# scipopt/SCIP-SDP

Measured on AMD Instinct MI355X. Metric: node-SDP solves/sec, dense block n x n with m vars (IPM iters/sec in iters_per_sec), higher is better.
Workload: dtype f64

## Files before the change

include/hipsdp.h:

```cpp
#ifndef HIPSDP_H
#define HIPSDP_H

#ifdef __cplusplus
extern "C" {
#endif

#define HIPSDP_API __attribute__((visibility("default")))

#define HIPSDP_OK             0
#define HIPSDP_ERR_NODEVICE   1
#define HIPSDP_ERR_HIP        2
#define HIPSDP_ERR_ARG        3
#define HIPSDP_ERR_NOMEM      4
#define HIPSDP_ERR_NUMERIC    5

#define HIPSDP_STATUS_OPTIMAL   0
#define HIPSDP_STATUS_DINF      1
#define HIPSDP_STATUS_DUNB      2
#define HIPSDP_STATUS_PDINF     3
#define HIPSDP_STATUS_ITERLIM   4
#define HIPSDP_STATUS_NUMERIC   5
#define HIPSDP_STATUS_TIMELIM   6
#define HIPSDP_STATUS_OBJLIM    7
#define HIPSDP_STATUS_UNSOLVED -1
// ... 27 lines not shown
   double dinf;
   double dabs;
   double gap;
   double mu;
   double tau, kappa;
   double solve_seconds;
   double schur_seconds;
   double schur_flops;
   int    schur_calls;
   int    chol_fail;
   int    warm_started;
   int    settings_used;
   double schur_flops_executed;
} hipsdp_info;

HIPSDP_API const char* hipsdp_last_error(void);
HIPSDP_API const char* hipsdp_version(void);
HIPSDP_API int  hipsdp_device_count(void);
HIPSDP_API void hipsdp_default_params(hipsdp_params* p);

HIPSDP_API int  hipsdp_create(hipsdp_solver** solver, int device);
HIPSDP_API void hipsdp_free(hipsdp_solver** solver);

HIPSDP_API int  hipsdp_set_shape(hipsdp_solver* solver, int m, int nblocks, const int* blocksizes, int q);
HIPSDP_API int  hipsdp_set_shape2(hipsdp_solver* solver, int m, int nblocks, const int* blocksizes, int q, const long long* nnz);
HIPSDP_API int  hipsdp_block_is_sparse(hipsdp_solver* solver, int block);
HIPSDP_API int  hipsdp_sparse_policy(hipsdp_solver* solver, int mode);
HIPSDP_API int  hipsdp_func_attr_sets(int device);
HIPSDP_API int  hipsdp_mem_info(int device, double* free_bytes, double* total_bytes);
HIPSDP_API int  hipsdp_set_obj(hipsdp_solver* solver, const double* b);
HIPSDP_API int  hipsdp_add_entries(hipsdp_solver* solver, int block, long long nnz, const int* var, const int* row, const int* col,
   const double* val);
HIPSDP_API int  hipsdp_master_define(hipsdp_solver* solver, int nvars, int nblocks, const int* blocksizes, const int* nblockvars);
HIPSDP_API int  hipsdp_master_add_entries(hipsdp_solver* solver, int block, long long nnz, const int* slot, const int* row, const int* col,
   const double* val);
HIPSDP_API int  hipsdp_master_add_vars(hipsdp_solver* solver, int block, int nslots, const int* nnz, const int* const* row,
   const int* const* col, const double* const* val);
HIPSDP_API int  hipsdp_master_gather(hipsdp_solver* solver, int engine_block, int master_block, int nactive, const int* slots,
   int nkept, const int* kept);
HIPSDP_API int  hipsdp_master_define2(hipsdp_solver* solver, int nvars, int nblocks, const int* blocksizes, const int* nblockvars,
   const long long* nnz);
HIPSDP_API int  hipsdp_master_block_is_sparse(hipsdp_solver* solver, int master_block);
HIPSDP_API int  hipsdp_master_gather_stats(hipsdp_solver* solver, long long* device_builds, long long* host_builds, long long* launches,
   long long* readbacks);
HIPSDP_API int  hipsdp_set_block_dense(hipsdp_solver* solver, int block, const double* A);
HIPSDP_API int  hipsdp_set_lp(hipsdp_solver* solver, const double* Dext);
HIPSDP_API int  hipsdp_block_device_ptr(hipsdp_solver* solver, int block, double** dptr);

HIPSDP_API int  hipsdp_set_start(hipsdp_solver* solver, const double* y, const double* const* X, const double* const* Z,
   const double* x, const double* z);

HIPSDP_API int  hipsdp_solve(hipsdp_solver* solver, const hipsdp_params* params, hipsdp_info* info);
HIPSDP_API int  hipsdp_gram_cache_stats(hipsdp_solver* solver, long long* hits, long long* misses);

HIPSDP_API int  hipsdp_solve_path(hipsdp_solver* solver);
HIPSDP_API long long hipsdp_solve1_solves(void);
HIPSDP_API long long hipsdp_solve1_fallbacks(void);
HIPSDP_API long long hipsdp_solve1_fallbacks_warm(void);
HIPSDP_API int hipsdp_solve1_debug_counts(unsigned int* counts2);
HIPSDP_API int  hipsdp_solve1_trace(hipsdp_solver* solver, double* out64, int maxrows, double* hist);

HIPSDP_API int hipsdp_solve_many(int count, hipsdp_solver* const* solvers, const hipsdp_params* params,
                                 hipsdp_info* infos, int* rcs);
HIPSDP_API int hipsdp_solve_many_stats(long long* launches, long long* problems);

HIPSDP_API int hipsdp_solve_objectives(hipsdp_solver* solver, int count, const double* B, const hipsdp_params* params,
                                       hipsdp_info* infos, double* Y, int* rcs);
HIPSDP_API int hipsdp_solve_objectives_stats(long long* calls, long long* launches, long long* problems);

HIPSDP_API int  hipsdp_get_y(hipsdp_solver* solver, double* y);
HIPSDP_API int  hipsdp_get_X(hipsdp_solver* solver, int block, double* X);
HIPSDP_API int  hipsdp_get_Z(hipsdp_solver* solver, int block, double* Z);
HIPSDP_API int  hipsdp_get_lp(hipsdp_solver* solver, double* x, double* z);
HIPSDP_API int  hipsdp_get_preoptimal(hipsdp_solver* solver, int* available, double* y, double* x);
HIPSDP_API int  hipsdp_get_preoptimal_X(hipsdp_solver* solver, int block, double* X);

HIPSDP_API int  hipsdp_check_y(hipsdp_solver* solver, const double* y, double* lmin, double* lpviol);
HIPSDP_API int  hipsdp_check_y_tol(hipsdp_solver* solver, const double* y, double tol, double* lmin, double* lpviol);

HIPSDP_API int  hipsdp_sync_flag(hipsdp_solver* solver, int* flag);

#define HIPSDP_NPHASES 7
HIPSDP_API int  hipsdp_set_profiling(hipsdp_solver* solver, int on);
HIPSDP_API int  hipsdp_get_phase_times(hipsdp_solver* solver, double* ms );
HIPSDP_API const char* hipsdp_phase_name(int phase);

HIPSDP_API int  hipsdp_eigencuts(hipsdp_solver* solver, int block, const double* y, double tol, int maxcuts, int* ncuts, double* eigvals,
                      double* coefs, double* lhs, double* vecs);
HIPSDP_API int hipsdp_eigencuts_all(hipsdp_solver* solver, const double* y, double tol, int maxcuts, int* ncuts, double* lmin,
                                    double* eigvals, double* coefs, double* lhs, double* vecs);
HIPSDP_API int hipsdp_eigencuts_all_stats(long long* calls, long long* launches, long long* readbacks);

#define HIPSDP_SPARSECUTS_MAXIT 10000
typedef struct hipsdp_sparsecut_opts {
   double tol;
   double feastol;
   double convtol;
   int    maxcuts;
   int    maxit;
} hipsdp_sparsecut_opts;
HIPSDP_API int hipsdp_sparsecuts_all(hipsdp_solver* solver, const double* y, const int* sizes, const hipsdp_sparsecut_opts* opts,
   int* ncuts, double* lmin, double* eigvals, double* coefs, double* lhs, double* vecs, int* iters, int* flags);
HIPSDP_API int hipsdp_sparsecuts_all_stats(long long* calls, long long* launches, long long* readbacks);

#define HIPSDP_SPARSECUTS_MAXN 512
HIPSDP_API int hipsdp_sparsecuts(hipsdp_solver* solver, int block, const double* y, int size, const hipsdp_sparsecut_opts* opts,
// ... 102 lines not shown
```

include/hipsdp_units.h:

```cpp
#ifndef HIPSDP_UNITS_H
#define HIPSDP_UNITS_H

#include "hipsdp.h"

#ifdef __cplusplus
extern "C" {
#endif

HIPSDP_API int  hipsdp_dgemm_selfcheck(int device, int M, int N, int K, int layB, int batch, int splitk, int flags, double beta,
   int* used_v2, long long* ndiff);
HIPSDP_API int  hipsdp_pass_at_unit(int device, int R, long long E, const double* A, const double* coef, double sa, const double* add, int split,
   double* out, int* chunks);
HIPSDP_API int  hipsdp_dgemm_selfcheck2(int device, int M, int N, int K, int layB, int batch, int splitk, int flags, double alpha, double beta,
   int reps, int* used, long long* ndiff, double* ms_tile, double* ms_fast);
HIPSDP_API int  hipsdp_gram_plan_info(int device, int M, long long K, int nslab, int* no, int* nd, int* nitems, double* span);
HIPSDP_API int  hipsdp_gram_selfcheck(int device, int M, long long K, int reps, int* used, double* maxdiff, long long* nrepro, double* ms_tile,
   double* ms_gram);
HIPSDP_API int  hipsdp_dgemm_selfcheck3(int device, int M, int N, int K, int layB, int batch, int splitk, int flags, double alpha, double beta,
   int reps, int* used, long long* ndiff, double* maxdiff, long long* nrepro, double* ms_tile, double* ms_fast);
HIPSDP_API int  hipsdp_tri_product_unit(int device, int mode, int M, int N, int K, int layB, int batch, int flags, const double* A,
   const double* B, double* Cio, int crows, int ldc, int* used);
HIPSDP_API int  hipsdp_tri_instance_force(int mode);
HIPSDP_API int  hipsdp_schur_identity_unit(int device, int m1, int n, const double* A, double ws_gbytes, int full_storage, double* Mx,
   double* flops);
// ... 30 lines not shown
   double* dZ);
HIPSDP_API int  hipsdp_tail_dirmat_unit(int device, int n, int fused, double s1, const double* Zinv, const double* X, const double* GZ, double* H,
   double* pk);
HIPSDP_API int  hipsdp_tail_sc_len(void);
HIPSDP_API int  hipsdp_tail_dir_unit(int device, int m, int n, int fused, const double* B, const double* H, const double* rhs2, const double* rp,
   const double* b, const double* u1, const double* u2, const double* par, double* sc, double* dy, double* dyt);
HIPSDP_API int  hipsdp_tail_dots_unit(int device, int m, int n, int fused, const double* a, const double* v, double* out);
HIPSDP_API int  hipsdp_trtri(int device, int n, const double* A, double* Linv);
HIPSDP_API int  hipsdp_lambda_min(int device, int n, const double* W, int steps, double* theta, double* resid);
HIPSDP_API int  hipsdp_lambda_min_scaled(int device, int n, const double* L, const double* D, int steps, double* theta, double* resid);
HIPSDP_API int  hipsdp_solve1_fits(int m, int q, int nblk, const int* ns);
HIPSDP_API int  hipsdp_solve1_class(int m, int nblk, const int* ns);
HIPSDP_API unsigned long long hipsdp_gram_gen_next(unsigned long long* counter);
HIPSDP_API int  hipsdp_gram_key_match_unit(int m_a, int nblk_a, const int* n_a, const int* form_a, const unsigned long long* gen_a,
   const long long* ws_a, int m_b, int nblk_b, const int* n_b, const int* form_b, const unsigned long long* gen_b, const long long* ws_b);
HIPSDP_API int  hipsdp_syev_many_unit(int device, int count, const int* ns, const double* A, double* lam, double* V, int* launches);
HIPSDP_API int  hipsdp_sparsecuts_unit(int device, int count, const int* ns, const double* Z, const double* v0, const double* maxeig,
   const int* sizes, const hipsdp_sparsecut_opts* opts, int* ncuts, double* eigvals, double* vecs, int* iters, int* flags);
HIPSDP_API int  hipsdp_sparsecuts_large_unit(int device, int n, const double* Z, const double* v0, double maxeig, int size,
   const hipsdp_sparsecut_opts* opts, int* ncuts, double* eigvals, double* vecs, int* iters, int* flags);
HIPSDP_API int  hipsdp_tridiag_unit(int device, int n, const double* A, double* d, double* e, double* Vrefl, double* tau);
HIPSDP_API int  hipsdp_tvec_unit(int device, int n, const double* d, const double* e, double* lam, double* Z);
HIPSDP_API int  hipsdp_sparse_dump_unit(hipsdp_solver* solver, int block, long long* counts, int* voff, int* vrow, int* vcol, double* vval,
   int* poff, int* prow, int* pcol, int* pvar, double* pval, int* foff, int* frow, int* fcol, double* fval, int* soff, int* srow, int* sent);
HIPSDP_API int  hipsdp_onevar_unit(int device, int n, int count, const double* Z, const double* A, const double* shift, const int* kind,
   const double* lb, const double* ub, double feastol, int maxevals, int* status, double* optval, double* lmin, double* grad, int* evals);
HIPSDP_API int  hipsdp_onevar_all_unit(int device, int count, const int* n, const double* Z, const double* A, const double* shift,
   const int* kind, const double* lb, const double* ub, double feastol, int maxevals, int mid_cap,
   int* status, double* optval, double* lmin, double* grad, int* evals);
HIPSDP_API int  hipsdp_onevar_large_unit(int device, int count, const int* n, const double* Z, const double* A, const double* shift,
   const int* kind, const double* lb, const double* ub, double feastol, int maxevals, int wg_cap, int chunk,
   int* status, double* optval, double* lmin, double* grad, int* evals, int* rounds);
HIPSDP_API int  hipsdp_objs_fanout_unit(int device, int count, int m, int q, int nblk, const int* ns, const double* B, const double* b_own,
   int have_start, const double* y, const double* x, const double* z, const double* XZ, int gap, double guard, long long* lane_len,
   long long* offs, double* lanes, int* launches);
HIPSDP_API int  hipsdp_small_dir_block_unit(int device, int n, double c, double s1, const double* X, const double* R, const double* E,
   const double* Zinv, int recorded, double* out, int* pending);
HIPSDP_API int  hipsdp_small_lp_rows_unit(int device, int q, int m1, const double* Dext, const double* v, int mode, double eta, double sigmu,
   const double* x, const double* z, const double* rd, const double* elp, int recorded, double* out1, double* out2, int* pending);
HIPSDP_API int  hipsdp_small_apply_A_unit(int device, int m1, int nblk, const int* n2, const double* A, const double* V, int q,
   const double* Dext, const double* vlp, int epi, double scal, const double* vin, int recorded, double* out, double* vout, int* pending);
HIPSDP_API int  hipsdp_small_elementwise_unit(int device, int n, const int* nn, const double* par, int use_elp, const double* in,
   const double* xs, int recorded, double* o_lp, double* o_mul, double* o_ext, double* ys, int* pending);
HIPSDP_API int  hipsdp_small_gemv_t_unit(int device, int R, long long E, long long lda, const double* A, const double* coef, double sa,
   int add_mode, const double* add, int recorded, double* out, int* pending);
HIPSDP_API int  hipsdp_reductions_unit(int device, int kind, int count, const int* len, const int* slot, const int* accumulate,
   const double* a, const double* b, const double* c, int nslots, const double* preset, int recorded, double* out, int* pending);
HIPSDP_API int  hipsdp_small_solve_unit(int device, int m, const double* M, int form, int nrhs, long long ld, double* rhs, double* u2,
   double* wt, int* pending, int* fail);
HIPSDP_API int  hipsdp_gemv_t3_unit(int device, int R, long long E, long long lda, const double* A, const double* c, int fused, double* out,
   int* took);
HIPSDP_API int  hipsdp_pass_a_unit(int device, int R, long long E, long long lda, const double* A, int nv, const double* V, int voff,
   long long wsdoubles, double* out, int* info);

#ifdef __cplusplus
}
#endif

#endif
```

scip-sdp_amd/binding.py:

```python
import ctypes as C
import os
import numpy as np

_HERE = os.path.dirname(os.path.abspath(__file__))
LIBPATH = os.environ.get("HIPSDP_LIB", os.path.join(_HERE, "lib", "libhipsdp.so"))

STATUS_NAMES = {0: "optimal", 1: "dual_infeasible", 2: "dual_unbounded", 3: "both_infeasible", 4: "iterlimit",
                5: "numeric", 6: "timelimit", 7: "objlimit", -1: "unsolved"}


class Params(C.Structure):
    _fields_ = [("gaptol", C.c_double), ("feastol", C.c_double), ("infeastol", C.c_double), ("objlimit", C.c_double),
                ("timelimit", C.c_double), ("gamma", C.c_double), ("ws_gbytes", C.c_double), ("maxiter", C.c_int),
                ("verbose", C.c_int), ("lanczos_steps", C.c_int), ("settings", C.c_int), ("pabstol", C.c_double), ("preoptgap", C.c_double)]


class Info(C.Structure):
    _fields_ = [("status", C.c_int), ("iterations", C.c_int), ("pobj", C.c_double), ("dobj", C.c_double),
                ("pinf", C.c_double), ("dinf", C.c_double), ("dabs", C.c_double), ("gap", C.c_double), ("mu", C.c_double),
                ("tau", C.c_double), ("kappa", C.c_double), ("solve_seconds", C.c_double), ("schur_seconds", C.c_double),
                ("schur_flops", C.c_double), ("schur_calls", C.c_int), ("chol_fail", C.c_int), ("warm_started", C.c_int),
                ("settings_used", C.c_int), ("schur_flops_executed", C.c_double)]


# ... 202 lines not shown
        A = np.zeros((self.m + 1, self.ns[k], self.ns[k]))
        _chk(self._l().hipsdp_get_block_dense(self.h, k, _dp(A)), "hipsdp_get_block_dense")
        return A

    def load_core(self, prob):
        self.set_shape(prob.m, [A.shape[1] for A in prob.blocks], prob.q)
        self.set_obj(prob.b)
        for k, A in enumerate(prob.blocks):
            self.set_block_dense(k, A)
        if prob.q:
            self.set_lp(np.concatenate([np.asarray(prob.c).reshape(-1, 1), prob.D], axis=1))

    def set_start(self, y, X, Z, x=None, z=None):
        y = _f64(y)
        Xs = [_f64(M) for M in X]
        Zs = [_f64(M) for M in Z]
        PX = (C.POINTER(C.c_double) * max(len(Xs), 1))(*[_dp(M) for M in Xs])
        PZ = (C.POINTER(C.c_double) * max(len(Zs), 1))(*[_dp(M) for M in Zs])
        xx = _f64(x if x is not None else np.zeros(max(self.q, 1)))
        zz = _f64(z if z is not None else np.zeros(max(self.q, 1)))
        _chk(self._l().hipsdp_set_start(self.h, _dp(y), PX, PZ, _dp(xx), _dp(zz)), "hipsdp_set_start")

    def solve(self, **kw):
        p = Params()
        self._l().hipsdp_default_params(C.byref(p))
        for k, v in kw.items():
            setattr(p, k, v)
        info = Info()
        _chk(self._l().hipsdp_solve(self.h, C.byref(p), C.byref(info)), "hipsdp_solve")
        return info

    def solve_objectives(self, B, **kw):
        B = _f64(B)
        if B.ndim != 2 or B.shape[1] != self.m:
            raise ValueError("solve_objectives: B must be count x %d" % self.m)
        n = B.shape[0]
        p = _params(kw)
        infos = (Info * max(n, 1))()
        rcs = (C.c_int * max(n, 1))()
        Y = np.zeros((n, self.m))
        rc = self._l().hipsdp_solve_objectives(self.h, n, _dp(B), C.byref(p), infos, _dp(Y), rcs)
        if rc != 0:
            raise RuntimeError("hipsdp_solve_objectives failed: rc=%d, per job %s (%s)" %
                               (rc, list(rcs)[:n], self._l().hipsdp_last_error().decode()))
        return [infos[i] for i in range(n)], Y

    def solve_path(self):
        return self._l().hipsdp_solve_path(self.h)

    def gram_cache_stats(self):
        hits = C.c_longlong(0)
        misses = C.c_longlong(0)
        _chk(self._l().hipsdp_gram_cache_stats(self.h, C.byref(hits), C.byref(misses)), "hipsdp_gram_cache_stats")
        return hits.value, misses.value

    def solve1_trace(self, rows=0):
        out = np.zeros(64)
        hist = np.zeros((max(rows, 1), 16))
        _chk(self._l().hipsdp_solve1_trace(self.h, _dp(out), rows, _dp(hist) if rows else None), "hipsdp_solve1_trace")
        return out, hist[:rows]

    def y(self):
        out = np.zeros(self.m)
        _chk(self._l().hipsdp_get_y(self.h, _dp(out)), "hipsdp_get_y")
        return out

    def X(self, k):
        out = np.zeros((self.ns[k], self.ns[k]))
        _chk(self._l().hipsdp_get_X(self.h, k, _dp(out)), "hipsdp_get_X")
        return out

    def Z(self, k):
        out = np.zeros((self.ns[k], self.ns[k]))
        _chk(self._l().hipsdp_get_Z(self.h, k, _dp(out)), "hipsdp_get_Z")
        return out

    def lp(self):
        x = np.zeros(self.q)
        z = np.zeros(self.q)
        _chk(self._l().hipsdp_get_lp(self.h, _dp(x), _dp(z)), "hipsdp_get_lp")
        return x, z

    def preoptimal(self):
        avail = C.c_int(0)
        y = np.zeros(max(1, self.m))
        x = np.zeros(max(1, self.q))
        _chk(self._l().hipsdp_get_preoptimal(self.h, C.byref(avail), _dp(y), _dp(x)), "hipsdp_get_preoptimal")
        if not avail.value:
            return None
        Xs = []
        for k, n in enumerate(self.ns):
            X = np.zeros((n, n))
            _chk(self._l().hipsdp_get_preoptimal_X(self.h, k, _dp(X)), "hipsdp_get_preoptimal_X")
            Xs.append(X)
        return y[:self.m], Xs, x[:self.q]

    def check_y(self, y, tol=0.0):
        y = _f64(y)
        lmin = np.zeros(max(1, len(self.ns)))
        viol = C.c_double(0.0)
        if tol > 0.0:
            _chk(self._l().hipsdp_check_y_tol(self.h, _dp(y), C.c_double(tol), _dp(lmin), C.byref(viol)), "hipsdp_check_y_tol")
        else:
            _chk(self._l().hipsdp_check_y(self.h, _dp(y), _dp(lmin), C.byref(viol)), "hipsdp_check_y")
        return lmin[:len(self.ns)], viol.value

# ... 516 lines not shown
def schur_sparse_unit2(n, m, coo, X, Zinv, kernel=-1, device=0):
    var, row, col, val = _coo_i32(coo)
    X = _f64(X); Zinv = _f64(Zinv)
    Mx = np.zeros((m + 1, m + 1))
    took = C.c_int(-7)
    _chk(ulib().hipsdp_schur_sparse_unit2(device, n, m, C.c_longlong(len(val)), _ip(var), _ip(row), _ip(col), _dp(val), _dp(X), _dp(Zinv),
                                          _dp(Mx), int(kernel), C.byref(took)), "hipsdp_schur_sparse_unit2")
    return Mx, took.value


def sparse_ops_unit(n, m, coo, V=None, coef=None, base=None, device=0):
    var, row, col, val = _coo_i32(coo)
    outA = outAT = None
    pV = pc = pb = pA = pAT = None
    if V is not None:
        V = _f64(V)
        assert V.shape == (n, n)
        outA = np.full(m, np.nan)
        pV, pA = _dp(V), _dp(outA)
    if coef is not None:
        coef = _f64(coef)
        assert coef.shape == (m + 1,)
        base = np.zeros((n, n)) if base is None else _f64(base)
        assert base.shape == (n, n)
        outAT = np.full((n, n), np.nan)
        pc, pb, pAT = _dp(coef), _dp(base), _dp(outAT)
    _chk(ulib().hipsdp_sparse_ops_unit(device, n, m, C.c_longlong(len(val)), _ip(var), _ip(row), _ip(col), _dp(val), pV, pc, pb, pA, pAT),
         "hipsdp_sparse_ops_unit")
    return outA, outAT


def schur_w(A, X, Z, device=0):
    A = _f64(A)
    m1, n = A.shape[0], A.shape[1]
    X = _f64(X)
    Z = _f64(Z)
    Mx = np.zeros((m1, m1))
    _chk(ulib().hipsdp_schur_w(device, m1, n, _dp(A), _dp(X), _dp(Z), _dp(Mx)), "hipsdp_schur_w")
    return Mx


def schur_form_unit(form, A, P, Q, parts=1, ws_gbytes=0.0, device=0):
    A = _f64(A)
    m1, n = A.shape[0], A.shape[1]
    P = _f64(P); Q = _f64(Q)
    assert A.shape == (m1, n, n) and P.shape == (n, n) and Q.shape == (n, n)
    Mx = np.zeros((m1, m1))
    used = (C.c_int * 3)(0, 0, 0)
    _chk(ulib().hipsdp_schur_form_unit(device, form, parts, m1, n, _dp(A), _dp(P), _dp(Q), C.c_double(ws_gbytes), _dp(Mx), used),
         "hipsdp_schur_form_unit")
    return Mx, tuple(used)


def schur_small_unit(As, Xs, Zinvs, Dext=None, x=None, z=None, fill=0.0, device=0):
    As = [_f64(a) for a in As]; Xs = [_f64(a) for a in Xs]; Zinvs = [_f64(a) for a in Zinvs]
    nblk, m1 = len(As), As[0].shape[0]
    ns = np.array([a.shape[1] for a in As], dtype=np.int32)
    for k in range(nblk):
        assert As[k].shape == (m1, ns[k], ns[k]) and Xs[k].shape == (ns[k], ns[k]) and Zinvs[k].shape == (ns[k], ns[k])
    q = 0 if Dext is None else int(np.shape(Dext)[0])
    if q > 0:
        Dext = _f64(Dext); x = _f64(x); z = _f64(z)
        assert Dext.shape == (q, m1) and x.shape == (q,) and z.shape == (q,)
    arr = C.POINTER(C.c_double) * nblk
    pA, pX, pZ = arr(*[_dp(a) for a in As]), arr(*[_dp(a) for a in Xs]), arr(*[_dp(a) for a in Zinvs])
    m = m1 - 1
    Mx = np.full((m1, m1), fill)
    Lm = np.full(max(m * m, 1), fill)
    dg = np.full(max(m, 1), fill)
    taken = C.c_int(-1)
    _chk(ulib().hipsdp_schur_small_unit(device, m1, nblk, _ip(ns), pA, pX, pZ, q, _dp(Dext) if q else None, _dp(x) if q else None,
                                        _dp(z) if q else None, _dp(Mx), _dp(Lm), _dp(dg), C.byref(taken)), "hipsdp_schur_small_unit")
    return taken.value, Mx, Lm[:m * m].reshape(m, m), dg[:m]


def gram_plan_info(M, K, nslab=64, device=0):
    no, nd, ni = C.c_int(0), C.c_int(0), C.c_int(0)
    sp = C.c_double(0.0)
    rc = ulib().hipsdp_gram_plan_info(device, M, C.c_longlong(K), nslab, C.byref(no), C.byref(nd), C.byref(ni), C.byref(sp))
    return (no.value, nd.value, ni.value, sp.value) if rc == 0 else None


def dgemm_selfcheck(M, N, K, layB=1, batch=1, splitk=1, flags=0, beta=0.0, device=0):
    used = C.c_int(0)
    nd = C.c_longlong(0)
    _chk(ulib().hipsdp_dgemm_selfcheck(device, M, N, K, layB, batch, splitk, flags, C.c_double(beta), C.byref(used), C.byref(nd)),
         "hipsdp_dgemm_selfcheck")
    return used.value, nd.value


def dgemm_selfcheck2(M, N, K, layB=1, batch=1, splitk=1, flags=0, alpha=1.0, beta=0.0, reps=0, device=0):
    used = C.c_int(0)
    nd = C.c_longlong(0)
    t0, t1 = C.c_double(0.0), C.c_double(0.0)
    _chk(ulib().hipsdp_dgemm_selfcheck2(device, M, N, K, layB, batch, splitk, flags, C.c_double(alpha), C.c_double(beta), reps,
                                       C.byref(used), C.byref(nd), C.byref(t0), C.byref(t1)), "hipsdp_dgemm_selfcheck2")
    return used.value, nd.value, t0.value, t1.value


def dgemm_selfcheck3(M, N, K, layB=1, batch=1, splitk=1, flags=0, alpha=1.0, beta=0.0, reps=0, device=0):
    used = C.c_int(0)
    nd, nr = C.c_longlong(0), C.c_longlong(0)
    md, t0, t1 = C.c_double(0.0), C.c_double(0.0), C.c_double(0.0)
    _chk(ulib().hipsdp_dgemm_selfcheck3(device, M, N, K, layB, batch, splitk, flags, C.c_double(alpha), C.c_double(beta), reps,
                                       C.byref(used), C.byref(nd), C.byref(md), C.byref(nr), C.byref(t0), C.byref(t1)), "hipsdp_dgemm_selfcheck3")
    return used.value, nd.value, md.value, nr.value, t0.value, t1.value
# ... 236 lines not shown
    _chk(ulib().hipsdp_small_elementwise_unit(device, n, _ip(nn), _dp(par), int(use_elp), _dp(vecs), _dp(xs), int(recorded), _dp(o_lp),
                                              _dp(o_mul), _dp(o_ext), _dp(ys), C.byref(pend)), "hipsdp_small_elementwise_unit")
    return o_lp, o_mul, o_ext, ys, pend.value


def small_gemv_t_unit(A, E, coef, sa, add, add_mode, recorded, device=0):
    A, coef = _f64(A), _f64(coef)
    R, lda = A.shape
    add = None if add is None else _f64(add)
    assert coef.size == R and 1 <= E <= lda and (add_mode == 0 or add.size == E)
    out, pend = np.zeros(E), C.c_int(-1)
    _chk(ulib().hipsdp_small_gemv_t_unit(device, R, C.c_longlong(E), C.c_longlong(lda), _dp(A), _dp(coef), C.c_double(sa), int(add_mode),
                                         _opt(add), int(recorded), _dp(out), C.byref(pend)), "hipsdp_small_gemv_t_unit")
    return out, pend.value


def reductions_unit(kind, lens, slots, accumulate, a, b, c, preset, recorded, device=0):
    lens, slots, accumulate = (np.ascontiguousarray(v, dtype=np.int32) for v in (lens, slots, accumulate))
    a, b, c, preset = _f64(a), _f64(b), _f64(c), _f64(preset)
    assert lens.size == slots.size == accumulate.size and a.size == b.size == c.size == int(lens.sum())
    out, pend = np.zeros(preset.size), C.c_int(-1)
    _chk(ulib().hipsdp_reductions_unit(device, int(kind), lens.size, _ip(lens), _ip(slots), _ip(accumulate), _dp(a), _dp(b), _dp(c),
                                       preset.size, _dp(preset), int(recorded), _dp(out), C.byref(pend)), "hipsdp_reductions_unit")
    return out, pend.value


def small_solve_unit(M, rhs, form, ld=None, device=0):
    M = _f64(M)
    m = M.shape[0]
    rhs = _f64(rhs).copy()
    pend, fail = C.c_int(-1), C.c_int(-1)
    if form == 0:
        nrhs, ld = rhs.shape
        _chk(ulib().hipsdp_small_solve_unit(device, m, _dp(M), 0, nrhs, C.c_longlong(ld), _dp(rhs), None, None, C.byref(pend),
                                            C.byref(fail)), "hipsdp_small_solve_unit")
        return rhs, pend.value, fail.value
    assert rhs.size == 2 * m
    u2, wt = np.zeros(m), np.zeros(m + 1)
    _chk(ulib().hipsdp_small_solve_unit(device, m, _dp(M), 1, 0, C.c_longlong(0), _dp(rhs), _dp(u2), _dp(wt), C.byref(pend),
                                        C.byref(fail)), "hipsdp_small_solve_unit")
    return rhs, u2, wt, fail.value


def gemv_t3_unit(A, E, c, fused, device=0):
    A, c = _f64(A), _f64(c)
    R, lda = A.shape
    assert c.shape == (3, R) and 1 <= E <= lda
    out, took = np.zeros((3, E)), C.c_int(-1)
    _chk(ulib().hipsdp_gemv_t3_unit(device, R, C.c_longlong(E), C.c_longlong(lda), _dp(A), _dp(c), int(fused), _dp(out), C.byref(took)),
         "hipsdp_gemv_t3_unit")
    return out, took.value


def pass_a_unit(A, E, V, voff=0, wsdoubles=0, device=0):
    A, V = _f64(A), _f64(V)
    R, lda = A.shape
    nv = V.shape[0]
    assert V.shape == (nv, E) and 1 <= E <= lda
    out = np.zeros((nv, R))
    info = np.zeros(2, dtype=np.int32)
    _chk(ulib().hipsdp_pass_a_unit(device, R, C.c_longlong(E), C.c_longlong(lda), _dp(A), nv, _dp(V), int(voff), C.c_longlong(wsdoubles),
                                   _dp(out), _ip(info)), "hipsdp_pass_a_unit")
    return out, int(info[0]), bool(info[1])


def trtri(A, device=0):
    A = _f64(A)
    Li = np.zeros_like(A)
    _chk(ulib().hipsdp_trtri(device, A.shape[0], _dp(A), _dp(Li)), "hipsdp_trtri")
    return Li


def lambda_min(W, steps=0, device=0):
    W = _f64(W)
    th = C.c_double(0.0)
    rs = C.c_double(0.0)
    _chk(ulib().hipsdp_lambda_min(device, W.shape[0], _dp(W), steps, C.byref(th), C.byref(rs)), "hipsdp_lambda_min")
    return th.value, rs.value


def syev(A, device=0):
    A = _f64(A)
    n = A.shape[0]
    lam = np.zeros(n)
    V = np.zeros((n, n))
    _chk(lib().hipsdp_syev(device, n, _dp(A), _dp(lam), _dp(V)), "hipsdp_syev")
    return lam, V


def syevx(A, il, iu, vectors=True, device=0):
    A = _f64(A)
    n = A.shape[0]
    k = max(0, iu - il + 1)
    lam = np.zeros(k)
    V = np.zeros((k, n)) if vectors else None
    _chk(lib().hipsdp_syevx(device, n, _dp(A), int(il), int(iu), _dp(lam), _dp(V) if vectors else None), "hipsdp_syevx")
    return lam, V


def syevx_below(A, bound, maxk, vectors=True, device=0):
    A = _f64(A)
    n = A.shape[0]
    lam = np.zeros(max(1, maxk))
    V = np.zeros((max(1, maxk), n)) if vectors else None
    cnt, nbelow = C.c_int(-1), C.c_int(-1)
    _chk(lib().hipsdp_syevx_below(device, n, _dp(A), C.c_double(bound), int(maxk), C.byref(cnt), C.byref(nbelow), _dp(lam),
# ... 97 lines not shown
```

scip-sdp_amd/csrc/chol.hip:

```cpp
#include "hs_kernels.h"
#include "hs_wave.h"
#include <cstdlib>

#define NB 64

#ifdef PD_TIMING
__device__ long long pd_tbuf[16];
__device__ int pd_tj0;
#define PD_T(idx) do { if ( threadIdx.x == 0 && j0 == pd_tj0 && blockIdx.x == (gridDim.x > 1 ? 1u : 0u) ) pd_tbuf[idx] = wall_clock64(); } while (0)
extern "C" __attribute__((visibility("default"))) int hipsdp_debug_pd_timing(int j0, long long* out)
{
   if ( out != NULL && hipMemcpyFromSymbol(out, HIP_SYMBOL(pd_tbuf), sizeof(long long) * 16) != hipSuccess )
      return 1;
   return hipMemcpyToSymbol(HIP_SYMBOL(pd_tj0), &j0, sizeof(int)) == hipSuccess ? 0 : 1;
}
#else
#define PD_T(idx) do { } while (0)
#endif

__device__ __forceinline__ void sqrt_and_rsqrt(double d, double y0, double* sd, double* isd)
{
   const double t = d * y0;
   const double e = fma(-t, y0, 1.0);
   const double p = fma(0.375, e, 0.5);
   const double y = fma(y0 * e, p, y0);
   double g = d * y;
   g = fma(fma(-g, g, d), 0.5 * y, g);
   *sd = g;
   *isd = y;
}

__device__ __forceinline__ void pd_wave_sync()
{
   __builtin_amdgcn_fence(__ATOMIC_RELEASE, "wavefront");
   __builtin_amdgcn_wave_barrier();
   __builtin_amdgcn_fence(__ATOMIC_ACQUIRE, "wavefront");
}

struct __attribute__((aligned(16))) dpair { double x, y; };
typedef double v4dc __attribute__((ext_vector_type(4)));

#define PD_LD (NB + 2)
#define PD_SMEM_BYTES ((2 * NB * PD_LD + 5 * NB) * (int) sizeof(double))

struct pd_ext
{
   const double* base;
   const double* dir;
   double        alpha;
   double*       Mout;
   double*       Linv;
   double*       Gram;
   int           set_flag;
   int           rule;
   int*          regmask;
   int           from_lds;
   int           nostore;
   double*       Lout;
};

__device__ __forceinline__ void pd_load_panel(double (&r)[16], const double (*W)[PD_LD], int lane, int c0, bool mine)
{
#pragma unroll
   for (int q = 0; q < 8; ++q)
   {
      dpair u = {0.0, 0.0};
      if ( mine )
         u = *reinterpret_cast<const dpair*>(&W[lane][c0 + 2 * q]);
      r[2 * q] = u.x;
      r[2 * q + 1] = u.y;
   }
}

template<bool CHECKED>
__device__ __forceinline__ bool pd_panel(double (&r)[16], const double (&thr)[16], const double* __restrict__ d0s, int lane, int c0, int nb, int j0,
   bool psd, double regtol, int rule, double (&isdo)[16], unsigned& fbits, int& bad, double* __restrict__ colb)
{
   bool special = false;
   fbits = 0u;
   double cprev[16], tprev = 0.0;
   double d = hs_lane(r[0], c0);
#pragma unroll
   for (int k = 0; k < 16; ++k)
   {
      const int gk = c0 + k;
      const double a = r[k];
      double sa = 0.0, sb = 0.0, sa2 = 0.0;
      if ( k + 1 < 16 )
      {
         sa = hs_lane(a, gk + 1);
         sb = hs_lane(r[k + 1], gk + 1);
      }
      if ( k + 2 < 16 )
         sa2 = hs_lane(a, gk + 2);
      double rc0 = __builtin_amdgcn_rcp(d);
      double y0 = __builtin_amdgcn_rsq(d);
// ... 577 lines not shown
         bufB[row][col] = v;
      }
   __syncthreads();
   ps_mma<true>(bufB, bufA, wave, lane, acc);
#pragma unroll
   for (int t = 0; t < 4; ++t)
#pragma unroll
      for (int rr = 0; rr < 4; ++rr)
      {
         const int row = 16 * wave + lk + 4 * rr, col = 16 * t + lr;
         if ( row < rows )
            Ark[(long long) row * lda + col] = forced[col] != 0.0 ? 0.0 : acc[t][rr];
      }
   PD_T(10);
}

template<int NBK>
__global__ void __launch_bounds__(256) k_potrf_step(double* __restrict__ A, long long lda, int n, int kb, int nblk,
   double* __restrict__ dinv, int* __restrict__ flag, const double* __restrict__ diag0, double regtol, pd_ext ext)
{
   ps_step_body<NBK>(A, lda, n, kb, nblk, dinv, flag, diag0, regtol, ext);
}

struct ps_job { double* A; double* dinv; int* flag; };
template<int NBK>
__global__ void __launch_bounds__(256) k_potrf_step_pair(ps_job J0, ps_job J1, long long lda, int n, int kb, int nblk, pd_ext ext)
{
   const ps_job J = blockIdx.y ? J1 : J0;
   ps_step_body<NBK>(J.A, lda, n, kb, nblk, J.dinv, J.flag, NULL, 1e-13, ext);
}

template<int NBK>
static int launch_potrf_step_pair(hipStream_t s, const ps_job* J, long long lda, int n, int kb, int nblk, const pd_ext& ext)
{
   static hs_attr_mask attr_done;
   HS_CALL( hs_func_max_lds(reinterpret_cast<const void*>(&k_potrf_step_pair<NBK>), PD_SMEM_BYTES, &attr_done) );
   const int nS = nblk - kb;
   const int t = nblk - kb - 1;
   const int nT = kb > 0 ? t * (t + 1) / 2 : 0;
   hipLaunchKernelGGL((k_potrf_step_pair<NBK>), dim3(nS + nT, 2), dim3(256), PD_SMEM_BYTES, s, J[0], J[1], lda, n, kb, nblk, ext);
   HS_LAUNCH_CHECK();
   return HS_OK;
}

template<int NBK>
static int launch_potrf_step(hipStream_t s, double* A, long long lda, int n, int kb, int nblk, double* dinv, int* flag,
   const double* diag0, const pd_ext& ext)
{
   static hs_attr_mask attr_done;
   HS_CALL( hs_func_max_lds(reinterpret_cast<const void*>(&k_potrf_step<NBK>), PD_SMEM_BYTES, &attr_done) );
   const int nS = nblk - kb;
   const int t = nblk - kb - 1;
   const int nT = kb > 0 ? t * (t + 1) / 2 : 0;
   hipLaunchKernelGGL((k_potrf_step<NBK>), dim3(nS + nT), dim3(256), PD_SMEM_BYTES, s, A, lda, n, kb, nblk, dinv, flag, diag0, 1e-13, ext);
   HS_LAUNCH_CHECK();
   return HS_OK;
}

template<int NBK>
static int launch_potrf_diag(hipStream_t s, double* Ajj, long long lda, int nb, int j0, double* dj, int* flag, const double* diag0,
   const pd_ext* extp = NULL)
{
   pd_ext ext = {NULL, NULL, 0.0, NULL, NULL, NULL, 0, 2, NULL};
   if ( extp != NULL )
      ext = *extp;
   static hs_attr_mask attr_done;
   HS_CALL( hs_func_max_lds(reinterpret_cast<const void*>(&k_potrf_diag<NBK>), PD_SMEM_BYTES, &attr_done) );
   hipLaunchKernelGGL((k_potrf_diag<NBK>), dim3(1), dim3(256), PD_SMEM_BYTES, s, Ajj, lda, nb, j0, dj, flag, diag0, 1e-13, ext);
   HS_LAUNCH_CHECK();
   return HS_OK;
}

int hs_potrf_small_ext(hipStream_t s, int n, double* L, double* dinv, int* flag, const double* base, const double* dir, double alpha,
   double* Mout, double* Linv, double* Gram, int set_flag)
{
   if ( n <= 0 )
      return HS_OK;
   if ( n > NB || base == NULL || (Gram != NULL && n > 32) )
      return HS_ERR_ARG;
   pd_ext ext = {base, dir, alpha, Mout, Linv, Gram, set_flag, 2, NULL};
   if ( n <= 16 )
      return launch_potrf_diag<16>(s, L, n, n, 0, dinv, flag, NULL, &ext);
   if ( n <= 32 )
      return launch_potrf_diag<32>(s, L, n, n, 0, dinv, flag, NULL, &ext);
   if ( n <= 48 )
      return launch_potrf_diag<48>(s, L, n, n, 0, dinv, flag, NULL, &ext);
   return launch_potrf_diag<64>(s, L, n, n, 0, dinv, flag, NULL, &ext);
}

template<int NBK>
static int launch_potrf_diag_pair(hipStream_t s, int n, const pd_job& J0, const pd_job& J1)
{
   static hs_attr_mask attr_done;
   HS_CALL( hs_func_max_lds(reinterpret_cast<const void*>(&k_potrf_diag_pair<NBK>), PD_SMEM_BYTES, &attr_done) );
   hipLaunchKernelGGL((k_potrf_diag_pair<NBK>), dim3(2), dim3(256), PD_SMEM_BYTES, s, J0, J1, (long long) n, n);
   HS_LAUNCH_CHECK();
   return HS_OK;
}

int hs_potrf_small_ext_pair(hipStream_t s, int n, double* const* L, double* const* dinv, int* const* flag, const double* const* base,
   const double* const* dir, double alpha, double* const* Mout, double* const* Linv, double* const* Gram, int set_flag)
{
   if ( n <= 0 )
      return HS_OK;
   if ( n > NB || base[0] == NULL || base[1] == NULL || ((Gram[0] != NULL || Gram[1] != NULL) && n > 32) )
      return HS_ERR_ARG;
   pd_job J[2];
   for (int k = 0; k < 2; ++k)
   {
      const pd_ext ext = {base[k], dir[k], alpha, Mout[k], Linv[k], Gram[k], set_flag, 2, NULL};
      J[k].A = L[k]; J[k].dinv = dinv[k]; J[k].flag = flag[k]; J[k].ext = ext;
   }
   if ( n <= 16 )
      return launch_potrf_diag_pair<16>(s, n, J[0], J[1]);
   if ( n <= 32 )
      return launch_potrf_diag_pair<32>(s, n, J[0], J[1]);
   if ( n <= 48 )
      return launch_potrf_diag_pair<48>(s, n, J[0], J[1]);
   return launch_potrf_diag_pair<64>(s, n, J[0], J[1]);
}

__global__ void k_zero_forced_cols(int rows, int nb, double* __restrict__ P, long long lda, const int* __restrict__ mask)
{
   for (long long e = (long long) blockIdx.x * blockDim.x + threadIdx.x; e < (long long) rows * nb; e += (long long) gridDim.x * blockDim.x)
   {
      const int r = (int) (e / nb), c = (int) (e - (long long) r * nb);
      if ( mask[c] )
         P[(long long) r * lda + c] = 0.0;
   }
}

static int g_potrf_force_v1 = 0;
int hs_potrf_force_v1(int on) { const int old = g_potrf_force_v1; g_potrf_force_v1 = on; return old; }

long long hs_potrf_dinv_len(int n)
{
   const long long nblk = n > 0 ? (n + NB - 1) / NB : 1;
   return (nblk > 1 ? 2 : 1) * nblk * NB * NB;
}

int hs_potrf(hipStream_t s, int n, double* A, double* dinv, int* flag, const double* diag0)
{
   return hs_potrf_psd(s, n, A, dinv, flag, diag0, NULL, 0);
}

int hs_potrf_pair(hipStream_t s, int n, const hs_potrf_job* jobs)
{
   if ( n <= 0 )
      return HS_OK;
   if ( jobs == NULL || jobs[0].A == NULL || jobs[1].A == NULL || jobs[0].A == jobs[1].A || jobs[0].dinv == jobs[1].dinv )
      return HS_ERR_ARG;
   const int nblk = (n + NB - 1) / NB;
   if ( nblk <= 1 || g_potrf_force_v1 )
   {
      HS_CALL( hs_potrf(s, n, jobs[0].A, jobs[0].dinv, jobs[0].flag, NULL) );
      return hs_potrf(s, n, jobs[1].A, jobs[1].dinv, jobs[1].flag, NULL);
   }
   const ps_job J[2] = {{jobs[0].A, jobs[0].dinv, jobs[0].flag}, {jobs[1].A, jobs[1].dinv, jobs[1].flag}};
   const pd_ext est = {NULL, NULL, 0.0, NULL, NULL, NULL, 0, 3, NULL, 0, 0, NULL};
   for (int b = 0; b < nblk; ++b)
   {
      const int nb = (n - b * NB) < NB ? (n - b * NB) : NB;
      if ( nb <= 16 )
         HS_CALL( launch_potrf_step_pair<16>(s, J, n, n, b, nblk, est) );
      else if ( nb <= 32 )
         HS_CALL( launch_potrf_step_pair<32>(s, J, n, n, b, nblk, est) );
      else
         HS_CALL( launch_potrf_step_pair<64>(s, J, n, n, b, nblk, est) );
   }
   return HS_OK;
}

int hs_potrf_psd(hipStream_t s, int n, double* A, double* dinv, int* flag, const double* diag0, int* regmask, int set_flag)
{
   if ( n <= 0 )
      return HS_OK;
   if ( diag0 != NULL && regmask == NULL && n > NB )
      return HS_ERR_ARG;
   static int rule = getenv("HIPSDP_PIVOT_RULE") != NULL ? atoi(getenv("HIPSDP_PIVOT_RULE")) : 3;
   pd_ext ext = {NULL, NULL, 0.0, NULL, NULL, NULL, (set_flag && n <= NB) ? 1 : 0, rule, regmask};
   const pd_ext* extp = ((diag0 != NULL && regmask != NULL) || ext.set_flag) ? &ext : NULL;
   const long long lda = n;
   const int nblk = (n + NB - 1) / NB;
   if ( nblk > 1 && !g_potrf_force_v1 )
   {
      pd_ext est = {NULL, NULL, 0.0, NULL, NULL, NULL, 0, rule, (diag0 != NULL) ? regmask : NULL, 0, 0, NULL};
      for (int b = 0; b < nblk; ++b)
      {
         const int nb = (n - b * NB) < NB ? (n - b * NB) : NB;
         if ( nb <= 16 )
            HS_CALL( launch_potrf_step<16>(s, A, lda, n, b, nblk, dinv, flag, diag0, est) );
         else if ( nb <= 32 )
            HS_CALL( launch_potrf_step<32>(s, A, lda, n, b, nblk, dinv, flag, diag0, est) );
         else
            HS_CALL( launch_potrf_step<64>(s, A, lda, n, b, nblk, dinv, flag, diag0, est) );
      }
      return HS_OK;
   }
   for (int b = 0; b < nblk; ++b)
   {
      const int j0 = b * NB;
      const int nb = (n - j0) < NB ? (n - j0) : NB;
      double* Ajj = A + (long long) j0 * lda + j0;
      double* dj = dinv + (long long) b * NB * NB;
      if ( nb <= 16 )
         HS_CALL( launch_potrf_diag<16>(s, Ajj, lda, nb, j0, dj, flag, diag0, extp) );
      else if ( nb <= 32 )
         HS_CALL( launch_potrf_diag<32>(s, Ajj, lda, nb, j0, dj, flag, diag0, extp) );
      else
         HS_CALL( launch_potrf_diag<64>(s, Ajj, lda, nb, j0, dj, flag, diag0, extp) );
      const int j1 = j0 + nb;
      const int rem = n - j1;
      if ( rem <= 0 )
         break;
      double* P = A + (long long) j1 * lda + j0;
      hs_gemm_args g1 = {rem, nb, nb, HS_KC, HS_KC, P, lda, 0, dj, NB, 0, P, lda, 0, 1.0, 0.0, 1, HS_GEMM_TILE64, 1, NULL};
      HS_CALL( hs_dgemm(s, &g1) );
      if ( diag0 != NULL && regmask != NULL )
      {
         long long blocks = ((long long) rem * nb + 255) / 256;
         if ( blocks > 1024 ) blocks = 1024;
         hipLaunchKernelGGL(k_zero_forced_cols, dim3((unsigned) blocks), dim3(256), 0, s, rem, nb, P, lda, regmask + j0);
         HS_LAUNCH_CHECK();
      }
      double* A22 = A + (long long) j1 * lda + j1;
      hs_gemm_args g2 = {rem, rem, nb, HS_KC, HS_KC, P, lda, 0, P, lda, 0, A22, lda, 0, -1.0, 1.0, 1, HS_GEMM_LOWER | HS_GEMM_TILE64, 1, NULL};
      HS_CALL( hs_dgemm(s, &g2) );
   }
   return HS_OK;
}

__global__ void k_copy_block(const double* __restrict__ src, long long lds_, double* __restrict__ dst, long long ldd, int rows, int cols,
// ... 740 lines not shown
```

scip-sdp_amd/csrc/dgemm2.hip:

```cpp
#include "hs_common.h"
#include <stdlib.h>
#include <map>
#include <mutex>
#include <utility>

typedef double v4d2 __attribute__((ext_vector_type(4)));
typedef __attribute__((address_space(3))) void* hs_lds_ptr;
typedef const __attribute__((address_space(1))) void* hs_gbl_ptr;

#define G2_BT   128
#define G2_BKS  8
#ifndef G2_NS
#define G2_NS   4
#endif
#ifndef G2_WGPC
#define G2_WGPC 2
#endif
#define G2_OPSZ (G2_BT * G2_BKS)
#define G2_SLOT (2 * G2_OPSZ)
#define G2_GPS  4
#ifndef G2_ABL
#define G2_ABL  0
#endif

// ... 1165 lines not shown
      run_band();
      store_item();
      cm0 = nm0; cn0 = nn0; cbz = nbz; cvalid = nvalid;
      ++gi;
   }
   g2_wait_vm<0>();
#ifdef G5_PROF
   if ( lane == 0 )
   {
      unsigned long long* o = g5_prof + ((long long) blockIdx.x * (WIDE ? 8 : 4) + wave) * 8;
      for (int i = 0; i < 7; ++i)
         o[i] = prof_acc[i];
      o[7] = __builtin_readcyclecounter() - prof_t0;
   }
#endif
}

#ifdef G5_PROF
extern "C" __attribute__((visibility("default"))) int hs_dgemm5_prof_read(unsigned long long* out)
{
   return hipMemcpyFromSymbol(out, HIP_SYMBOL(g5_prof), sizeof(unsigned long long) * 512 * 4 * 8) == hipSuccess ? 0 : 1;
}
#endif

static int g2_disabled = 0;
static int g2_taken = 0;
static int g5_taken = 0;
static int g5_wide_mode = -1;
static int g5_wide_taken = 0;

int hs_dgemm2_enable(int on)
{
   g2_disabled = on ? 0 : 1;
   return __atomic_load_n(&g2_taken, __ATOMIC_RELAXED);
}

int hs_dgemm2_paired_taken(void)
{
   return __atomic_load_n(&g5_taken, __ATOMIC_RELAXED);
}

int hs_dgemm2_wide_force(int mode)
{
   if ( mode >= -1 && mode <= 1 )
      g5_wide_mode = mode;
   return __atomic_load_n(&g5_wide_taken, __ATOMIC_RELAXED);
}

int hs_dgemm2_tri5_forced(void)
{
   return g5_wide_mode >= 0;
}

static unsigned int* g5_counters(hipStream_t stream)
{
   static std::mutex mu;
   static std::map<std::pair<int, hipStream_t>, unsigned int*> tab;
   int dev = 0;
   if ( hipGetDevice(&dev) != hipSuccess )
      return NULL;
   std::lock_guard<std::mutex> lk(mu);
   auto it = tab.find(std::make_pair(dev, stream));
   if ( it != tab.end() )
      return it->second;
   unsigned int* q = NULL;
   if ( hipMalloc((void**) &q, 64) != hipSuccess )
      return NULL;
   tab[std::make_pair(dev, stream)] = q;
   return q;
}

int hs_dgemm2_tri5_eligible(const hs_gemm_args* a)
{
   const bool triA = (a->flags & HS_GEMM_A_LOWTRI) != 0, triB = (a->flags & HS_GEMM_B_LOWTRI) != 0;
   return triA != triB && a->splitk <= 1 && !(a->flags & (HS_GEMM_LOWER | HS_GEMM_UPPER | HS_GEMM_A_UPTRI))
      && !(triB && a->layB != HS_MC);
}

int hs_dgemm2_tri5_wide(const hs_gemm_args* a)
{
   if ( !hs_dgemm2_tri5_eligible(a) )
      return 0;
   if ( g5_wide_mode >= 0 )
      return g5_wide_mode;
   const bool triB = (a->flags & HS_GEMM_B_LOWTRI) != 0;
   if ( !((G5_WIDE_TRI >> (triB ? 0 : 1)) & 1) )
      return 0;
   const long long panels = triB ? (a->N + G2_BT - 1) / G2_BT : (a->M + G2_BT - 1) / G2_BT;
   const long long wtiles = triB ? (a->M + 2 * G2_BT - 1) / (2 * G2_BT) : (long long) ((a->N + 2 * G2_BT - 1) / (2 * G2_BT)) * a->batch;
   if ( !triB && 2 * ((a->N + 2 * G2_BT - 1) / (2 * G2_BT)) != (a->N + G2_BT - 1) / G2_BT )
      return 0;
   return panels >= 4 && panels * wtiles >= 256LL * G5_WIDE_MIN_ITEMS;
}

int hs_dgemm2_try(hipStream_t stream, const hs_gemm_args* a, int kchunk)
{
   if ( g2_disabled )
      return 0;
   if ( a->layA != HS_KC || (a->flags & (HS_GEMM_UPPER)) )
      return 0;
   if ( (a->lda & 1) || (a->ldb & 1) || (a->strideA & 1) || (a->strideB & 1) || (a->K & 1) || a->K < 16 )
      return 0;
   if ( (((uintptr_t) a->A) & 15) || (((uintptr_t) a->B) & 15) )
      return 0;
   if ( a->layB == HS_MC && ((a->N & 1) || a->N < 2) )
      return 0;
   if ( (a->flags & HS_GEMM_LOWER) && a->M != a->N )
      return 0;
   if ( a->splitk > 1 && (kchunk & 15) )
      return 0;
   const long long tm = (a->M + G2_BT - 1) / G2_BT, tn = (a->N + G2_BT - 1) / G2_BT;
   const long long ntile = (a->flags & HS_GEMM_LOWER) ? tm * (tm + 1) / 2 : tm * tn;
   const long long nz = a->splitk > 1 ? a->splitk : a->batch;
   const long long total = ntile * nz;
   if ( total < 384 && !(g5_wide_mode >= 0 && hs_dgemm2_tri5_eligible(a)) )
      return 0;
   int grid = 256 * G2_WGPC;
   const int Wx = grid / 8;
   int rotdiv = 0;
   if ( !(a->flags & HS_GEMM_LOWER) )
   {
      if ( (a->flags & HS_GEMM_B_LOWTRI) && tn > 1 && (Wx % tn) == 0 )
         rotdiv = (int) (Wx / tn);
      else if ( (a->flags & (HS_GEMM_A_LOWTRI | HS_GEMM_A_UPTRI)) && tm > 1 && (Wx % (tm * tn)) == 0 )
         rotdiv = (int) (Wx / (tm * tn));
   }
   const size_t smem = (size_t) G2_NS * G2_SLOT * sizeof(double);
   const bool triA = (a->flags & HS_GEMM_A_LOWTRI) != 0, triB = (a->flags & HS_GEMM_B_LOWTRI) != 0;
   if ( hs_dgemm2_tri5_eligible(a) )
   {
      static hs_attr_mask attr5[6];
      const int wide = hs_dgemm2_tri5_wide(a);
      const int inst5 = (triB ? 0 : (a->layB == HS_MC ? 1 : 2)) + 3 * wide;
      const size_t smem5 = (size_t) G5_NS * (wide ? 3 * G2_OPSZ : G2_SLOT) * sizeof(double);
      const void* fn5 = NULL;
      switch ( inst5 )
      {
      case 0: fn5 = reinterpret_cast<const void*>(&hs_dgemm5_kernel<HS_MC, 1, 0>); break;
      case 1: fn5 = reinterpret_cast<const void*>(&hs_dgemm5_kernel<HS_MC, 2, 0>); break;
      case 2: fn5 = reinterpret_cast<const void*>(&hs_dgemm5_kernel<HS_KC, 2, 0>); break;
      case 3: fn5 = reinterpret_cast<const void*>(&hs_dgemm5_kernel<HS_MC, 1, 1>); break;
      case 4: fn5 = reinterpret_cast<const void*>(&hs_dgemm5_kernel<HS_MC, 2, 1>); break;
      default: fn5 = reinterpret_cast<const void*>(&hs_dgemm5_kernel<HS_KC, 2, 1>); break;
      }
      if ( hs_func_max_lds(fn5, (int) smem5, &attr5[inst5]) != HS_OK )
         return -HS_ERR_HIP;
      unsigned int* ctr = g5_counters(stream);
      if ( ctr == NULL || hipMemsetAsync(ctr, 0, 64, stream) != hipSuccess )
         return -HS_ERR_HIP;
      hs_gemm_args a5 = *a;
      a5.flags |= G5_F_NT | G5_F_SETS | G5_F_PAIRS;
      const long long tm5 = triB && wide ? (a->M + 2 * G2_BT - 1) / (2 * G2_BT) : tm;
      const long long tn5 = !triB && wide ? (a->N + 2 * G2_BT - 1) / (2 * G2_BT) : tn;
      const long long ntile5 = tm5 * tn5, total5 = ntile5 * nz;
      const int grid5 = wide ? 256 : grid;
      switch ( inst5 )
      {
      case 0: hipLaunchKernelGGL((hs_dgemm5_kernel<HS_MC, 1, 0>), dim3(grid5), dim3(256), smem5, stream, a5, ntile5, total5, ctr); break;
      case 1: hipLaunchKernelGGL((hs_dgemm5_kernel<HS_MC, 2, 0>), dim3(grid5), dim3(256), smem5, stream, a5, ntile5, total5, ctr); break;
      case 2: hipLaunchKernelGGL((hs_dgemm5_kernel<HS_KC, 2, 0>), dim3(grid5), dim3(256), smem5, stream, a5, ntile5, total5, ctr); break;
      case 3: hipLaunchKernelGGL((hs_dgemm5_kernel<HS_MC, 1, 1>), dim3(grid5), dim3(512), smem5, stream, a5, ntile5, total5, ctr); break;
      case 4: hipLaunchKernelGGL((hs_dgemm5_kernel<HS_MC, 2, 1>), dim3(grid5), dim3(512), smem5, stream, a5, ntile5, total5, ctr); break;
      default: hipLaunchKernelGGL((hs_dgemm5_kernel<HS_KC, 2, 1>), dim3(grid5), dim3(512), smem5, stream, a5, ntile5, total5, ctr); break;
      }
      if ( hipGetLastError() != hipSuccess )
         return -HS_ERR_HIP;
      (void) __atomic_add_fetch(&g2_taken, 1, __ATOMIC_RELAXED);
      (void) __atomic_add_fetch(&g5_taken, 1, __ATOMIC_RELAXED);
      if ( wide )
         (void) __atomic_add_fetch(&g5_wide_taken, 1, __ATOMIC_RELAXED);
      return 1;
   }
   const int il = triA != triB ? (triB ? 1 : 2) : 0;
   static hs_attr_mask attr_done[6];
   const int inst = (a->layB == HS_KC ? 0 : 3) + il;
   const void* fn = NULL;
   switch ( inst )
   {
   case 0: fn = reinterpret_cast<const void*>(&hs_dgemm2_kernel<HS_KC, 0>); break;
   case 1: fn = reinterpret_cast<const void*>(&hs_dgemm2_kernel<HS_KC, 1>); break;
   case 2: fn = reinterpret_cast<const void*>(&hs_dgemm2_kernel<HS_KC, 2>); break;
   case 3: fn = reinterpret_cast<const void*>(&hs_dgemm2_kernel<HS_MC, 0>); break;
   case 4: fn = reinterpret_cast<const void*>(&hs_dgemm2_kernel<HS_MC, 1>); break;
   default: fn = reinterpret_cast<const void*>(&hs_dgemm2_kernel<HS_MC, 2>); break;
   }
   if ( hs_func_max_lds(fn, (int) smem, &attr_done[inst]) != HS_OK )
      return -HS_ERR_HIP;
   switch ( inst )
   {
   case 0: hipLaunchKernelGGL((hs_dgemm2_kernel<HS_KC, 0>), dim3(grid), dim3(256), smem, stream, *a, kchunk, ntile, total, rotdiv); break;
   case 1: hipLaunchKernelGGL((hs_dgemm2_kernel<HS_KC, 1>), dim3(grid), dim3(256), smem, stream, *a, kchunk, ntile, total, rotdiv); break;
   case 2: hipLaunchKernelGGL((hs_dgemm2_kernel<HS_KC, 2>), dim3(grid), dim3(256), smem, stream, *a, kchunk, ntile, total, rotdiv); break;
   case 3: hipLaunchKernelGGL((hs_dgemm2_kernel<HS_MC, 0>), dim3(grid), dim3(256), smem, stream, *a, kchunk, ntile, total, rotdiv); break;
   case 4: hipLaunchKernelGGL((hs_dgemm2_kernel<HS_MC, 1>), dim3(grid), dim3(256), smem, stream, *a, kchunk, ntile, total, rotdiv); break;
   default: hipLaunchKernelGGL((hs_dgemm2_kernel<HS_MC, 2>), dim3(grid), dim3(256), smem, stream, *a, kchunk, ntile, total, rotdiv); break;
   }
   if ( hipGetLastError() != hipSuccess )
      return -HS_ERR_HIP;
   (void) __atomic_add_fetch(&g2_taken, 1, __ATOMIC_RELAXED);
   return 1;
}
```

scip-sdp_amd/csrc/gram.hip:

```cpp
#include "hs_common.h"
#include <stdlib.h>
#include <stdio.h>
#include <map>
#include <mutex>
#include <utility>
#include <tuple>
#include <vector>
#include <queue>
#include <algorithm>
#include <functional>

typedef double gr_v4d __attribute__((ext_vector_type(4)));
typedef __attribute__((address_space(3))) void* gr_lds_ptr;
typedef const __attribute__((address_space(1))) void* gr_gbl_ptr;

#define GR_BT   128
#define GR_BKS  8
#define GR_NS   4
#define GR_OPSZ (GR_BT * GR_BKS)
#define GR_SLOT (2 * GR_OPSZ)
#define GR_GPS  4
#define GR_UNI(x) __builtin_amdgcn_readfirstlane(x)

__device__ __attribute__((aligned(16))) double hs_gr_zero[2] = {0.0, 0.0};
// ... 263 lines not shown
            for (int i = 0; i < 4; ++i)
#pragma unroll
               for (int r = 0; r < 4; ++r)
               {
                  const int row = m0 + wm * 64 + 16 * i + (lane >> 4) + 4 * r;
                  if ( row < g.M )
                  {
                     double* cr = C + (long long) row * g.M + n0 + wn * 64 + (lane & 15);
#pragma unroll
                     for (int j = 0; j < 4; ++j)
                        cr[16 * j] = acc[4 * i + j][r];
                  }
               }
         }
         else
         {
#pragma unroll
            for (int k = 0; k < 9; ++k)
            {
               const int rs = dlo[k] ? wave : 7 - wave;
#pragma unroll
               for (int r = 0; r < 4; ++r)
               {
                  const int row = m0 + 16 * rs + (lane >> 4) + 4 * r;
                  const int col = m0 + 16 * dcol[k] + (lane & 15);
                  if ( row < g.M && col < g.M )
                     C[(long long) row * g.M + col] = acc[k][r];
               }
            }
         }
#pragma unroll
         for (int i = 0; i < 16; ++i)
            acc[i] = (gr_v4d){0.0, 0.0, 0.0, 0.0};
      }
      __syncthreads();
   }
}

__global__ void hs_gram_reduce_kernel(int M, int no, int nd, const double* __restrict__ ws, double* __restrict__ C, long long ldc, double alpha, double beta)
{
   const long long MM = (long long) M * M;
   for (long long e = (long long) blockIdx.x * blockDim.x + threadIdx.x; e < MM; e += (long long) gridDim.x * blockDim.x)
   {
      const int r = (int) (e / M), c = (int) (e - (long long) r * M);
      if ( c > r )
         continue;
      const int ns = (r / GR_BT == c / GR_BT) ? nd : no;
      double s = 0.0;
      for (int k = 0; k < ns; ++k)
         s += ws[(long long) k * MM + e];
      double* q = C + (long long) r * ldc + c;
      *q = beta != 0.0 ? alpha * s + beta * (*q) : alpha * s;
   }
}

namespace {

struct GramPlan
{
   std::vector<gram_item> items;
   std::vector<int> off;
   int no, nd;
   double span;
   double executed;
   gram_item* dev;
   int* devoff;
};

#define GR_DIAG_COST 0.72

bool gr_make_plan(GramPlan& P, int tm, long long K, int so, int sd)
{
   const int noff = tm * (tm - 1) / 2;
   const double cd = GR_DIAG_COST;
   if ( so < 1 || sd < 1 )
      return false;
   long long lo = (K + so - 1) / so, ld = (K + sd - 1) / sd;
   lo = ((lo + GR_BKS - 1) / GR_BKS) * GR_BKS;
   ld = ((ld + GR_BKS - 1) / GR_BKS) * GR_BKS;
   if ( (long long) (so - 1) * lo + 8 * GR_BKS > K || (long long) (sd - 1) * ld + 8 * GR_BKS > K )
      return false;
   std::vector<gram_item> all;
   for (int s = 0; s < so; ++s)
      for (int i = 1; i < tm; ++i)
         for (int j = 0; j < i; ++j)
         {
            gram_item it = {i, j, (int) (s * lo), (int) ((s + 1) * lo < K ? (s + 1) * lo : K), s, 0};
            all.push_back(it);
         }
   for (int s = 0; s < sd; ++s)
      for (int i = 0; i < tm; ++i)
      {
         gram_item it = {i, i, (int) (s * ld), (int) ((s + 1) * ld < K ? (s + 1) * ld : K), s, 0};
         all.push_back(it);
      }
   (void) noff;
   std::stable_sort(all.begin(), all.end(), [](const gram_item& a, const gram_item& b) { return a.k0 < b.k0; });
   auto cost = [&](const gram_item& it) { return (it.ti == it.tj ? cd : 1.0) * (double) (it.k1 - it.k0) / (double) K; };
   double total = 0.0;
   P.executed = 0.0;
   for (const gram_item& it : all)
   {
      total += cost(it);
      P.executed += 2048.0 * (double) ((it.k1 - it.k0 + GR_BKS - 1) / GR_BKS) * (it.ti == it.tj ? 72.0 : 128.0);
   }
   P.items.clear();
// ... 60 lines not shown
         return;
      cand.span += penalty;
      if ( best == NULL || cand.span < best->span )
      {
         if ( best == NULL )
            best = new GramPlan();
         *best = cand;
      }
   };
   const int noff = ntile - tm;
   for (int so = 1; so <= nslab && (long long) noff * so + tm <= 512; ++so)
      for (int sd = (so + 1) / 2; sd <= so && (long long) noff * so + (long long) tm * sd <= 512; ++sd)
         consider(gr_make_plan(cand, tm, K, so, sd), 0.24 * ((double) so * noff + (double) sd * tm) / (double) K);
   if ( best != NULL )
   {
      const int sold = hs_dgemm_pick_xcd_slices(ntile, K);
      const double oldspan = (double) (((long long) ntile * sold + 511) / 512) / (double) sold;
      if ( best->span * 1.03 > oldspan || best->items.size() < 256 )
      {
         delete best;
         best = NULL;
      }
   }
   if ( best != NULL )
   {
      gram_item* d = NULL;
      int* doff = NULL;
      if ( hipMalloc((void**) &d, best->items.size() * sizeof(gram_item)) != hipSuccess
         || hipMemcpy(d, best->items.data(), best->items.size() * sizeof(gram_item), hipMemcpyHostToDevice) != hipSuccess
         || hipMalloc((void**) &doff, 513 * sizeof(int)) != hipSuccess
         || hipMemcpy(doff, best->off.data(), 513 * sizeof(int), hipMemcpyHostToDevice) != hipSuccess )
      {
         if ( d != NULL ) (void) hipFree(d);
         if ( doff != NULL ) (void) hipFree(doff);
         delete best;
         return NULL;
      }
      best->dev = d;
      best->devoff = doff;
   }
   tab[key] = best;
   return best;
}

}

static int gr_taken = 0;

int hs_gram_taken(void)
{
   return __atomic_load_n(&gr_taken, __ATOMIC_RELAXED);
}

int hs_gram_try(hipStream_t stream, int M, long long K, const double* W, long long ldw, double* C, long long ldc, double alpha, double beta,
   double* ws, int nslab, double* executed)
{
   if ( ws == NULL || nslab < 2 || M < 256 || K < 16384 )
      return 0;
   if ( (ldw & 1) || (K & 1) || (((uintptr_t) W) & 15) || K > 2000000000LL )
      return 0;
   if ( nslab > 64 ) nslab = 64;
   GramPlan* P = gr_plan(M, K, nslab);
   if ( P == NULL || P->dev == NULL || P->items.size() < 256 )
      return 0;
   gram_args g;
   g.W = W; g.ldw = ldw; g.M = M; g.ws = ws; g.items = P->dev; g.off = P->devoff;
   static hs_attr_mask attr_done;
   const size_t smem = (size_t) GR_NS * GR_SLOT * sizeof(double);
   if ( hs_func_max_lds(reinterpret_cast<const void*>(&hs_gram_kernel), (int) smem, &attr_done) != HS_OK )
      return -HS_ERR_HIP;
   hipLaunchKernelGGL(hs_gram_kernel, dim3(512), dim3(256), smem, stream, g);
   if ( hipGetLastError() != hipSuccess )
      return -HS_ERR_HIP;
   {
      int blocks = (int) (((long long) M * M + 255) / 256);
      if ( blocks > 2048 ) blocks = 2048;
      hipLaunchKernelGGL(hs_gram_reduce_kernel, dim3(blocks), dim3(256), 0, stream, M, P->no, P->nd, ws, C, ldc, alpha, beta);
      if ( hipGetLastError() != hipSuccess )
         return -HS_ERR_HIP;
   }
   if ( executed != NULL )
      *executed = P->executed;
   (void) __atomic_add_fetch(&gr_taken, 1, __ATOMIC_RELAXED);
   return 1;
}

int hs_gram_plan_info(int M, long long K, int nslab, int* no, int* nd, int* nitems, double* span)
{
   GramPlan* P = gr_plan(M, K, nslab > 64 ? 64 : nslab);
   if ( P == NULL )
      return 0;
   *no = P->no; *nd = P->nd; *nitems = (int) P->items.size(); *span = P->span;
   return 1;
}
```

scip-sdp_amd/csrc/hs_common.h:

```cpp
#ifndef HS_COMMON_H
#define HS_COMMON_H

#include <hip/hip_runtime.h>
#include <stddef.h>
#include <stdint.h>

#define HS_OK            0
#define HS_ERR_NODEVICE  1
#define HS_ERR_HIP       2
#define HS_ERR_ARG       3
#define HS_ERR_NOMEM     4
#define HS_ERR_NUMERIC   5

#define HS_HIP(call)                                                                       \
   do {                                                                                    \
      hipError_t hs_e_ = (call);                                                           \
      if ( hs_e_ != hipSuccess ) {                                                         \
         hs_record_hip_error(hs_e_, #call, __FILE__, __LINE__);                            \
         return (hs_e_ == hipErrorOutOfMemory) ? HS_ERR_NOMEM : HS_ERR_HIP;                \
      }                                                                                    \
   } while (0)

#define HS_CALL(call)                                                                      \
   do {                                                                                    \
// ... 10 lines not shown
         return HS_ERR_HIP;                                                                \
      }                                                                                    \
   } while (0)

void hs_record_hip_error(hipError_t e, const char* what, const char* file, int line);
const char* hs_last_error(void);

struct hs_attr_mask { unsigned long long bits[2]; };
int hs_func_max_lds(const void* fn, int bytes, hs_attr_mask* done);
int hs_func_attr_sets(int device);
int hs_device_cus(void);

int hs_pool_alloc(void** p, size_t bytes);
void hs_pool_free(void* p);
void hs_pool_trim(void);

#define HS_KC 0
#define HS_MC 1

#define HS_GEMM_LOWER     1
#define HS_GEMM_A_LOWTRI  2
#define HS_GEMM_B_LOWTRI  4
#define HS_GEMM_A_UPTRI 256
#define HS_GEMM_XCD       8
#define HS_GEMM_TILE64  128
#define HS_GEMM_NOFAST   64
#define HS_GEMM_UPPER    32
#define HS_GEMM_REMAP    16
int hs_dgemm_pick_xcd_slices(long long ntile, long long K);

struct hs_gemm_args
{
   int            M, N, K;
   int            layA, layB;
   const double*  A;
   long long      lda;
   long long      strideA;
   const double*  B;
   long long      ldb;
   long long      strideB;
   double*        C;
   long long      ldc;
   long long      strideC;
   double         alpha, beta;
   int            batch;
   int            flags;
   int            splitk;
   double*        ws;
};

int hs_dgemm(hipStream_t stream, const hs_gemm_args* args);
int hs_dgemm2_try(hipStream_t stream, const hs_gemm_args* args, int kchunk);
int hs_dgemm2_enable(int on);
int hs_dgemm2_paired_taken(void);
int hs_dgemm2_wide_force(int mode);
int hs_dgemm2_tri5_forced(void);
int hs_gram_taken(void);

int hs_gram_try(hipStream_t stream, int M, long long K, const double* W, long long ldw, double* C, long long ldc, double alpha, double beta,
   double* ws, int nslab, double* executed);
int hs_gram_plan_info(int M, long long K, int nslab, int* no, int* nd, int* nitems, double* span);

int hs_dgemm3_try(hipStream_t stream, const hs_gemm_args* args);

double hs_mfma_flops_total(void);
void   hs_mfma_flops_add(double flops);
int hs_dgemm2_tri5_eligible(const hs_gemm_args* a);
int hs_dgemm2_tri5_wide(const hs_gemm_args* a);
double hs_gemm_executed_flops(const hs_gemm_args* a, int BT, int kstage, int kchunk, int persistent);

int hs_dgemm_pick_splitk(int M, int N, int K, int lowerOnly);

#endif
```

scip-sdp_amd/csrc/hs_gram_cache.h:

```cpp
#ifndef HS_GRAM_CACHE_H
#define HS_GRAM_CACHE_H

#define HS_GRAM_FORM_FULL   1
#define HS_GRAM_FORM_PACKED 2
#define HS_GRAM_MAXBLK 64

struct hs_gram_key
{
   int valid;
   int m, nblk;
   int n[HS_GRAM_MAXBLK];
   int form[HS_GRAM_MAXBLK];
   unsigned long long gen[HS_GRAM_MAXBLK];
   long long kws_len, chunk_cols;
   int ws_full;
};

static inline unsigned long long hs_gen_next(unsigned long long* counter)
{
   return ++*counter;
}

static inline void hs_gram_key_clear(hs_gram_key* k)
{
   k->valid = 0;
   k->m = 0;
   k->nblk = 0;
   k->kws_len = k->chunk_cols = 0;
   k->ws_full = 0;
}

static inline int hs_gram_key_make(hs_gram_key* k, int m, int nblk, const int* n, const int* form, const unsigned long long* gen,
   long long kws_len, long long chunk_cols, int ws_full)
{
   hs_gram_key_clear(k);
   if ( m < 0 || nblk < 1 || nblk > HS_GRAM_MAXBLK )
      return 0;
   for (int b = 0; b < nblk; ++b)
   {
      if ( n[b] < 1 || gen[b] == 0 || (form[b] != HS_GRAM_FORM_FULL && form[b] != HS_GRAM_FORM_PACKED) )
         return 0;
      k->n[b] = n[b];
      k->form[b] = form[b];
      k->gen[b] = gen[b];
   }
   k->m = m;
   k->nblk = nblk;
   k->kws_len = kws_len;
   k->chunk_cols = chunk_cols;
   k->ws_full = ws_full;
   k->valid = 1;
   return 1;
}

static inline int hs_gram_key_match(const hs_gram_key* have, const hs_gram_key* want)
{
   if ( !have->valid || !want->valid || have->m != want->m || have->nblk != want->nblk || have->kws_len != want->kws_len
      || have->chunk_cols != want->chunk_cols || have->ws_full != want->ws_full )
      return 0;
   for (int b = 0; b < have->nblk; ++b)
      if ( have->n[b] != want->n[b] || have->form[b] != want->form[b] || have->gen[b] != want->gen[b] )
         return 0;
   return 1;
}

#endif
```

scip-sdp_amd/csrc/hs_kernels.h:

```cpp
#ifndef HS_KERNELS_H
#define HS_KERNELS_H

#include "hs_common.h"
#include "hs_cut_plan.h"
#include <vector>

int hs_fill(hipStream_t s, double* p, long long n, double v);
int hs_set_identity(hipStream_t s, double* A, int n, double v);
int hs_copy(hipStream_t s, double* dst, const double* src, long long n);
int hs_axpy(hipStream_t s, long long n, double a, const double* x, double* y);
int hs_scale_add(hipStream_t s, long long n, double a, const double* x, double b, const double* y, double* out);
struct hs_trial_job { double* V; const double* dV; double* Vs; double* L; };
int hs_trial_pair(hipStream_t s, long long n, double alpha, int first, const hs_trial_job* jobs);
int hs_mirror_lower(hipStream_t s, double* A, int n, long long lda);
int hs_symmetrize(hipStream_t s, double* A, int n);
int hs_transpose(hipStream_t s, int n, const double* src, double* dst);

int hs_gemv_n(hipStream_t s, int R, long long E, const double* A, long long lda, int nv, const double* const* V,
   double* out, long long ldo, double* ws, long long wsdoubles);
int hs_gemv_t(hipStream_t s, int R, long long E, const double* A, long long lda, const double* coef, double sa,
   const double* add, double* out);

int hs_gemv_t_chunks(int R, long long E);
int hs_gemv_t_ws(hipStream_t s, int R, long long E, const double* A, long long lda, const double* coef, double sa,
// ... 29 lines not shown
#define HS_DOT_SLOT_DOUBLES 256
#define HS_DOT_SLOTS 4
#define HS_RED_WS_DOUBLES (HS_DOT_SLOTS * HS_DOT_SLOT_DOUBLES)
int hs_dot_deferred(hipStream_t s, long long n, const double* a, const double* b, double* out, int accumulate, double* ws, int slot);
int hs_absmax(hipStream_t s, long long n, const double* a, double* out, int accumulate, double* ws);
int hs_ratio_min(hipStream_t s, long long n, const double* x, const double* d, double* out, int accumulate, double* ws);

#define HS_SMALL_N 48
int hs_dir_block_small(hipStream_t s, int n, double c, const double* X, const double* R, const double* E, const double* Zinv,
   double s1, double* out);
int hs_dirmat(hipStream_t s, int n, double s1, const double* Zinv, const double* X, const double* GZ, double* H);
int hs_dirmat_pack(hipStream_t s, int n, double s1, const double* Zinv, const double* X, const double* GZ, double* H, double* pk);

int hs_lp_dir(hipStream_t s, int q, double sigmu, double eta, const double* x, const double* z, const double* rd_or_dz,
   const double* elp, double* out);
int hs_lp_scale_rows(hipStream_t s, int q, int cols, const double* x, const double* z, const double* D, double* S);
int hs_vec_mul(hipStream_t s, long long n, const double* a, const double* b, double* out);
int hs_lp_s0(hipStream_t s, int q, const double* x, const double* z, const double* beta, double* out, int accumulate, double* ws);

int hs_pack_rows(hipStream_t s, int m1, int n, long long Lp, const double* A, double* Apk);
int hs_packed_diag(hipStream_t s, int m1, int n, int ldd, long long Lp, const double* Apk, double* D);
int hs_sub_lower(hipStream_t s, int n, const double* S, double* C);
int hs_pack_weighted(hipStream_t s, int n, const double* V, double* pk);
int hs_unpack_sym(hipStream_t s, int n, const double* pk, double sa, const double* add, double* out);
int hs_unpack_sym3(hipStream_t s, int n, int cnt, const double* const* pk, double* const* out);
int hs_unpack_dz_combine(hipStream_t s, int n, const double* pk, const double* P2, const double* sc, int idtau, double eta, const double* Rd,
   double* dZ);
int hs_zero_upper(hipStream_t s, double* A, int n);

struct hs_schur_ws
{
   double*   T;
   double*   U;
   double*   K;
   double*   V;
   long long capT, capV;
   long long chunk_cols;
   long long n2;
   long long kws_len;
   int       full;
   double*   U2;
   double*   V2;
   void*     evP[2];
   void*     evX[2];
   void*     ev_g2;
   int       (*after_g1)(void*);
   void*     after_g1_arg;
};
int  hs_schur_ws_alloc(hs_schur_ws* w, int m1, long long n2max, double budget_gb);
void hs_schur_ws_free(hs_schur_ws* w);
int  hs_schur_U(hipStream_t s, int m1, int n, const double* A, const double* X, const double* Zinv, double* Mx,
   hs_schur_ws* w, int j_begin, int j_end);
int  hs_schur_W(hipStream_t s, int m1, int n, const double* A, const double* R, const double* G, double* Mx, hs_schur_ws* w);
int  hs_schur_W_identity(hipStream_t s, int m1, int n, const double* A, double* Mx, hs_schur_ws* w);
int  hs_schur_W_identity_range(hipStream_t s, int m1, int n, const double* A, long long k0, long long k1, double* Mx, hs_schur_ws* w);
int  hs_schur_W_identity_packed(hipStream_t s, int m1, int n, const double* Apk, long long Lp, double* Mx, hs_schur_ws* w);
int  hs_schur_identity_packed_fits(const hs_schur_ws* w, int m1, int n);

int  hs_schur_Urows(hipStream_t s, int m1, int n, const double* A, const double* X, const double* Zinv, double* Mx,
   hs_schur_ws* w, int r_begin, int r_end);
void hs_shard_rows(int m1, int nranks, int rank, int* chunk_rows, int* first_begin, int* second_begin);
int  hs_schur_Wcols(hipStream_t s, int m1, int n, const double* A, const double* R, const double* G, double* Mx, hs_schur_ws* w,
   int c0, int cw);
void hs_shard_cols(int m1, int n, int nranks, int rank, int* c_begin, int* c_width);
int  hs_schur_Wvar(hipStream_t s, void* comm, int rank, int nranks, int m1, int n, const double* A, const double* R, const double* G,
   double* Mx, hs_schur_ws* w, int c0, int cw);
int  hs_schur_ws_alloc_var(hs_schur_ws* w, int m1, int nranks, int n, int cwmax);
int  hs_schur_ws_alloc_var_overlap(hs_schur_ws* w);
int  hs_schur_Wvar_all(hipStream_t s, hipStream_t sc, void* comm, int rank, int nranks, int m1, int n, const double* A, const double* R,
   const double* G, double* Mx, hs_schur_ws* w, int cwmax, int overlap);
void hs_var_rows(int m1, int nranks, int rank, int* r0, int* r1);
void hs_var_wrows(int n, int nranks, int rank, int* q0, int* q1);
int  hs_alltoall(void* comm, const double* send, double* recv, const long long* cnt, hipStream_t stream);
int  hs_allreduce_sum(void* comm, double* buf, long long count, hipStream_t stream);
int  hs_mirror_upper(hipStream_t s, double* A, int n, long long lda);
int  hs_allgather_inplace(void* comm, double* buf, long long count_per_rank, int rank, hipStream_t stream);
int  hs_allgather(void* comm, const double* send, double* recv, long long count_per_rank, hipStream_t stream);

struct hs_sparse
{
   int        n, m;
   long long  nnz;
   int*       voff;
   int*       vrow;
   int*       vcol;
   double*    vval;
   long long  npos;
   int*       poff;
   int*       prow;
   int*       pcol;
   int*       pvar;
   double*    pval;
   long long  nfull, nslots;
   int*       foff;
   int*       frow;
   int*       fcol;
   double*    fval;
   int*       soff;
   int*       srow;
   int*       sent;
   double*    Tc;
   int        borrowed;
};
int  hs_sp_prefers_sparse(int n, int m, long long nnz);
int  hs_sp_build(hs_sparse** out, int n, int m, long long nnz, const int* var, const int* row, const int* col, const double* val);
void hs_sp_free(hs_sparse* sp);
long long hs_sp_nnz(const hs_sparse* sp);
int  hs_sp_apply_A(hipStream_t s, const hs_sparse* sp, const double* V, double* out_var1);
int  hs_sp_apply_AT(hipStream_t s, const hs_sparse* sp, const double* coef, double* out);
int  hs_sp_schur(hipStream_t s, const hs_sparse* sp, const double* X, const double* Zinv, double* Mx);
int  hs_sp_schur_ex(hipStream_t s, const hs_sparse* sp, const double* X, const double* Zinv, double* Mx, int kernel, int* took);
int  hs_sp_expand(hipStream_t s, const hs_sparse* sp, double* A);

struct hs_spm;
int  hs_spm_create(hs_spm** out, int N, int S);
void hs_spm_free(hs_spm* M);
int  hs_spm_size(const hs_spm* M);
int  hs_spm_slots(const hs_spm* M);
int  hs_spm_add(hs_spm* M, long long nnz, const int* slot, int oneslot, const int* row, const int* col, const double* val);
int  hs_spm_gather_sparse(hipStream_t s, hs_spm* M, int n, int m, int nactive, const int* act, const int* kept, hs_sparse** out,
   long long* launches, long long* readbacks);
int  hs_spm_gather_dense(hipStream_t s, hs_spm* M, int n, int nactive, const int* dact, const int* dinv, double* A, long long* launches);
struct hipsdp_solver;
int  hs_solver_sparse_block(struct hipsdp_solver* s, int block, const hs_sparse** sp);

struct hs_dir_tail_args { int m, q, K; const int* n; const double* const* B; const double* const* H; const double* beta; const double* hl;
   const double* rhs2; const double* rp; const double* b; double* u1; const double* u2; double* dy; double* dyt; double* sc; double* red_ws;
   const double* dinvm; const double* Lm; double eta, rg, sigmu, tau, kappa, etk; };
int hs_ipm_dir_tail(hipStream_t st, const hs_dir_tail_args* a, int tail, int fuse_solve);
int hs_ipm_after_solve2(hipStream_t st, int m, const double* rhs2, double* u2, double* wt, const double* u1, double* e2, double* e1, int fused);
int hs_ipm_dz_combine(hipStream_t st, long long n2, double* dZ, const double* P2, const double* sc, double eta, const double* Rd);
int hs_ipm_sc_dtau(void);
int hs_ipm_sc_len(int nblocks);

int hs_potrf(hipStream_t s, int n, double* A, double* dinv, int* flag, const double* diag0);
long long hs_potrf_dinv_len(int n);
int hs_potrf_psd(hipStream_t s, int n, double* A, double* dinv, int* flag, const double* diag0, int* regmask, int set_flag);
struct hs_potrf_job { double* A; double* dinv; int* flag; };
int hs_potrf_pair(hipStream_t s, int n, const hs_potrf_job* jobs);
int hs_trtri(hipStream_t s, int n, const double* L, const double* dinv, double* Linv, double* tmp);
int hs_potrf_small_ext_pair(hipStream_t s, int n, double* const* L, double* const* dinv, int* const* flag, const double* const* base,
   const double* const* dir, double alpha, double* const* Mout, double* const* Linv, double* const* Gram, int set_flag);
int hs_potrf_small_ext(hipStream_t s, int n, double* L, double* dinv, int* flag, const double* base, const double* dir, double alpha,
   double* Mout, double* Linv, double* Gram, int set_flag);
int hs_schur_small(hipStream_t s, int m1, int nblk, const int* n, const double* const* A, const double* const* X,
   const double* const* Zinv, int q, const double* Dext, const double* x, const double* z, double* Mx, double* Lm, double* diagM);
int hs_trsv(hipStream_t s, int n, const double* L, const double* dinv, int nrhs, double* rhs, long long ldr, int mode);
long long hs_trsv_sync_ws(int n);
int hs_trsv_sync_init(hipStream_t s, int n, int* sync_ws, int* epoch);
int hs_trsv_sync(hipStream_t s, int n, const double* L, const double* dinv, int nrhs, double* rhs, long long ldr, int mode,
   int* sync_ws, int* epoch);

int hs_lanczos_lmin(hipStream_t s, int n, const double* W, int maxsteps, double* res, double* ws);
long long hs_lanczos_ws(int n, int maxsteps);
#define HS_STEP_MAXJOBS 32
struct hs_step_jobs { int nblk; int n[HS_STEP_MAXJOBS]; const double* L0[HS_STEP_MAXJOBS]; const double* D0[HS_STEP_MAXJOBS];
   const double* L1[HS_STEP_MAXJOBS]; const double* D1[HS_STEP_MAXJOBS]; double* res0[HS_STEP_MAXJOBS]; double* res1[HS_STEP_MAXJOBS]; };
int hs_steplen_small_multi(hipStream_t s, const hs_step_jobs* P, int maxsteps);
int hs_lmin_exact_multi(hipStream_t st, const hs_step_jobs* P);
int hs_lanczos_scaled_small(hipStream_t s, int n, int maxsteps, const double* L0, const double* D0, const double* L1, const double* D1,
   double* res0, double* res1);
int hs_lmin_scaled_tiny(hipStream_t s, int n, const double* L0, const double* D0, const double* L1, const double* D1, double* res0,
   double* res1);
int hs_lanczos_lmin2(hipStream_t s, int n, const double* W0, const double* W1, int maxsteps, double* res0, double* res1,
   double* ws0, double* ws1, int* rot, unsigned long long* dsync, int nwipe);
long long hs_lanczos_sync_words(void);
int hs_lanczos_sync_reset(hipStream_t s, unsigned long long* dsync, int* rot);

long long hs_syev_small_scratch(int n);
int hs_syev_small_dev(hipStream_t st, int n, const double* A, double* lam, double* V, double* scratch);
struct hs_eig_job { int n; int pad; const double* in; double* ws; };
long long hs_syev_many_vecpos(int n);
int hs_syev_many_class(int n);
int hs_syev_small_many(hipStream_t st, int count, const hs_eig_job* hjobs, const hs_eig_job* jobs, int* launches);

int hs_psd_project_one(int device, int n, int nnz, const int* row, const int* col, const double* val, double minev,
   double epsilon, int mode, int cap, int* nnz_out, int* rowout, int* colout, double* valout);

#define HS_EC_DENSE  0
#define HS_EC_PACKED 1
#define HS_EC_SPARSE 2
struct hs_sp_view { long long nnz, npos; const int *voff, *vrow, *vcol; const double* vval; const int *poff, *prow, *pcol, *pvar; const double* pval; };
void hs_sp_get_view(const hs_sparse* sp, hs_sp_view* v);
struct hs_ec_job
{
   int n, form, blk, pad;
   long long ld;
   const double* A;
   hs_sp_view sp;
   double* Z;
// ... 463 lines not shown
```

scip-sdp_amd/csrc/ipm.hip:

```cpp
#include "hs_kernels.h"
#include "hs_gram_cache.h"
#include "hs_sp_master.h"
#include "../../include/hipsdp.h"
#include <rocprofiler-sdk-roctx/roctx.h>
#include <vector>
#include <atomic>
#include <utility>
#include <functional>
#include <chrono>
#include <algorithm>
#include <cmath>
#include <cassert>
#include <cstdio>
#include <cstdlib>
#include <cstring>

enum
{
   SC_AX0 = 0,
   SC_DOBJ,
   SC_XZ,
   SC_RP2,
   SC_RD2,
   SC_RDLPMAX,
// ... 168 lines not shown
   long long gemv_ws_len;
   int* flags;
   hs_schur_ws sws;
   bool schur_mode_U, schur_mode_rows;
   bool schur_mode_cols;
   int  schur_sim_shards;
   bool schur_mode_forced;
   double* Mgather;
   long long mx_rows;
   int nsc;
   bool shaped, solved, have_start;
   int last_status;
   double sol_scale;
   hipEvent_t ev0, ev1;
   int master_nvars;
   std::vector<int> master_sizes;
   std::vector<int> master_slots;
   std::vector<double*> master_A;
   std::vector<hs_spm*> master_sp;
   long long mg_device_builds, mg_host_builds, mg_launches, mg_readbacks;
   void* comm; int rank, nranks;
   double* passg;
   int shard_passes;
   int shardA_req;
   int var_cw;
   bool var_overlap;
   bool shardA;
   int a_r0, a_r1;
   hipsdp_params par;
   PhaseClock pc;
   bool clk_on; unsigned long long* clk_buf; int clk_n; double clk_ghz; hipStream_t clk_stream;
   double* s1_ws;
   long long s1_ws_len;
   double* s1_host;
   double* s1_host_dev;
   bool s1_sol_host;
   bool zero_b, zero_D;
   char* arena_h; char* arena_d; size_t arena_cap, stage_off; bool stage_pending;
   int m_alloc, q_alloc;
   int ncmd;
   hipEvent_t cmd_ev;
   bool cmd_inflight;
   unsigned long long s1_seq;
   int s1_last;
   double* ln_dev; long long ln_dev_len;
   double* ln_host; double* ln_host_dev; long long ln_host_len;
   unsigned long long ln_seq;
   void* stage_h[2]; void* stage_d[2]; hipEvent_t stage_ev[2]; long long stage_cap;
   CutWs cw;
   unsigned long long a_gen_next;
   double* gc_M; long long gc_len; bool gc_nomem;
   hs_gram_key gc_key;
   long long gc_hits, gc_misses;
};

static void a_written(hipsdp_solver* s, Block& B)
{
   B.apk_valid = false;
   B.A_gen = hs_gen_next(&s->a_gen_next);
}

void hs_comm_phase(int phase);

static void phase_mark(hipsdp_solver* s, int ph)
{
   if ( s->pc.open >= 0 )
      (void) roctxRangePop();
   s->pc.open = ph;
   if ( ph >= 0 )
      (void) roctxRangePushA(g_phase_names[ph]);
   if ( !s->pc.on )
      return;
   hipEvent_t e = NULL;
   if ( !s->pc.pool.empty() )
   {
      e = s->pc.pool.back();
      s->pc.pool.pop_back();
   }
   else if ( hipEventCreate(&e) != hipSuccess )
      return;
   if ( hipEventRecord(e, s->stream) == hipSuccess )
      s->pc.marks.push_back(std::make_pair(ph, e));
   else
      s->pc.pool.push_back(e);
}

static void phase_finish(hipsdp_solver* s)
{
   for (size_t i = 0; i + 1 < s->pc.marks.size(); ++i)
   {
      float ms = 0.f;
      const int ph = s->pc.marks[i].first;
      if ( ph >= 0 && hipEventElapsedTime(&ms, s->pc.marks[i].second, s->pc.marks[i + 1].second) == hipSuccess )
         s->pc.ms[ph] += (double) ms;
   }
   for (auto& mk : s->pc.marks)
      s->pc.pool.push_back(mk.second);
   s->pc.marks.clear();
}

extern "C" const char* hipsdp_phase_name(int phase)
{
   return phase >= 0 && phase < PH_COUNT ? g_phase_names[phase] : "";
}

extern "C" int hipsdp_set_profiling(hipsdp_solver* s, int on)
{
// ... 168 lines not shown
      s->zero_b = false;
   }
   if ( s->zero_D )
   {
      HS_CALL( stage_zero(s, s->Dext, (long long) s->q * (s->m + 1)) );
      s->zero_D = false;
   }
   return HIPSDP_OK;
}
static int stage_sync(hipsdp_solver* s)
{
   if ( s != NULL && (s->zero_b || s->zero_D) )
      HS_CALL( flush_zeros(s) );
   if ( s != NULL && s->ncmd > 0 )
      HS_CALL( flush_cmds(s) );
   if ( s != NULL && s->stage_pending )
   {
      HS_HIP( hipStreamSynchronize(s->stream) );
      s->stage_pending = false;
      s->stage_off = 0;
      s->cmd_inflight = false;
   }
   return HIPSDP_OK;
}

static void free_sparse(Block& B)
{
   if ( B.sp != NULL ) hs_sp_free(B.sp);
   B.sp = NULL;
   delete B.sph;
   B.sph = NULL;
}

static void free_problem(hipsdp_solver* s)
{
   if ( s->stream != NULL ) (void) hipStreamSynchronize(s->stream);
   if ( s->stream2 != NULL ) (void) hipStreamSynchronize(s->stream2);
   for (auto& B : s->blk)
   {
      double* ptrs[] = {B.Aown, B.A0sep, B.X, B.Z, B.Rd, B.Lz, B.LzInv, B.Zinv, B.Lx, B.LxInv, B.B, B.H, B.G, B.GZ, B.dXa, B.dZa, B.dX, B.dZ,
         B.E, B.W, B.T1, B.dinvz, B.dinvx, B.Xs, B.Zs, B.Apkown, B.pkv, B.T2, B.W2, B.Xpre, B.P2, B.pk3};
      for (double* p : ptrs) dfree(p);
      free_sparse(B);
   }
   s->blk.clear();
   double* ptrs[] = {s->b, s->Dext, s->y, s->x, s->z, s->yt, s->dyt, s->wt, s->AX, s->AH, s->tmpe, s->rp, s->rd, s->tmpq, s->hl,
      s->beta, s->elp, s->dxa, s->dza, s->dx, s->dz, s->xs, s->zs, s->ys, s->rhs2, s->cvec, s->u2, s->dy, s->dya, s->Mx, s->Lm,
      s->dinvm, s->Slp, s->sc, s->red_ws, s->gemv_ws, s->lan_ws, s->lan_ws2};
   for (double* p : ptrs) dfree(p);
   hs_schur_ws_free(&s->sws);
   if ( s->gc_M != NULL ) (void) hipFree(s->gc_M);
   s->gc_M = NULL; s->gc_len = 0; s->gc_nomem = false;
   hs_gram_key_clear(&s->gc_key);
   if ( s->ln_dev != NULL ) (void) hipFree(s->ln_dev);
   if ( s->ln_host != NULL ) (void) hipHostFree(s->ln_host);
   s->ln_dev = NULL; s->ln_host = NULL; s->ln_host_dev = NULL; s->ln_dev_len = 0; s->ln_host_len = 0;
   dfree(s->Mgather);
   s->Mgather = NULL;
   dfree(s->passg);
   s->passg = NULL;
   dfree(s->trsv_ws);
   s->trsv_ws = NULL;
   dfree(s->gemvt_ws);
   s->gemvt_ws = NULL;
   s->gemvt_ws_len = 0;
   if ( s->lan_sync != NULL )
      (void) hipFree(s->lan_sync);
   s->lan_sync = NULL;
   dfree(s->regmask);
   s->regmask = NULL;
   dfree(s->pre_y); dfree(s->pre_x);
   s->pre_y = s->pre_x = NULL;
   s->pre_valid = false;
   s->b = s->Dext = s->y = s->x = s->z = s->yt = s->dyt = s->wt = s->AX = s->AH = s->tmpe = s->rp = s->rd = s->tmpq = s->hl = NULL;
   s->beta = s->elp = s->dxa = s->dza = s->dx = s->dz = s->xs = s->zs = s->ys = s->u1 = s->rhs2 = s->cvec = s->u2 = s->dy = s->dya = NULL;
   s->Mx = s->Lm = s->dinvm = s->Slp = s->sc = s->red_ws = s->gemv_ws = s->lan_ws = s->lan_ws2 = NULL;
   s->flags = NULL;
   s->shaped = false;
   s->solved = false;
}

extern "C" int hipsdp_create(hipsdp_solver** out, int device)
{
   g_err[0] = 0;
   int nd = hipsdp_device_count();
   if ( nd <= 0 )
   {
      set_err("no HIP device available (hipsdp has no CPU fallback)");
      return HIPSDP_ERR_NODEVICE;
   }
   if ( device < 0 || device >= nd )
      return HIPSDP_ERR_ARG;
   HS_HIP( hipSetDevice(device) );
   hipsdp_solver* s = new hipsdp_solver();
   memset((void*) &s->par, 0, sizeof(s->par));
   s->device = device;
   s->m = s->q = 0;
   s->b = s->Dext = s->y = s->x = s->z = NULL;
   s->shaped = s->solved = s->have_start = false;
   s->comm = NULL; s->rank = 0; s->nranks = 1;
   s->shardA_req = 0; s->shardA = false; s->a_r0 = 0; s->a_r1 = 1;
   s->passg = NULL;
   s->shard_passes = getenv("HIPSDP_SHARD_PASSES") != NULL ? atoi(getenv("HIPSDP_SHARD_PASSES")) : -1;
   s->master_nvars = 0;
   s->mg_device_builds = s->mg_host_builds = s->mg_launches = s->mg_readbacks = 0;
   s->Mgather = NULL;
   s->schur_mode_rows = false;
   s->schur_mode_cols = false; s->schur_sim_shards = 0;
   s->sws.T = s->sws.U = s->sws.K = s->sws.V = s->sws.U2 = s->sws.V2 = NULL;
   s->sws.evP[0] = s->sws.evP[1] = s->sws.evX[0] = s->sws.evX[1] = NULL; s->sws.ev_g2 = NULL; s->sws.after_g1 = NULL; s->sws.after_g1_arg = NULL;
   s->flags = NULL;
   s->hsc = NULL;
   s->hsc_dev = NULL;
   s->pub_seq = 0;
   s->hsc_cap = 0;
   s->clk_on = false; s->clk_buf = NULL; s->clk_n = 0; s->clk_ghz = 0.0; s->clk_stream = NULL;
   s->s1_ws = NULL; s->s1_ws_len = 0; s->s1_host = NULL; s->s1_host_dev = NULL; s->s1_seq = 0; s->s1_last = 0; s->s1_sol_host = false; s->zero_b = false; s->zero_D = false;
   s->arena_h = NULL; s->arena_d = NULL; s->arena_cap = 0; s->stage_off = 0; s->stage_pending = false; s->ncmd = 0; s->cmd_ev = NULL; s->cmd_inflight = false; s->m_alloc = 0; s->q_alloc = 0;
   s->ln_dev = NULL; s->ln_dev_len = 0; s->ln_host = NULL; s->ln_host_dev = NULL; s->ln_host_len = 0; s->ln_seq = 0;
   s->trsv_ws = NULL;
   s->a_gen_next = 0; s->gc_M = NULL; s->gc_len = 0; s->gc_nomem = false; s->gc_hits = s->gc_misses = 0;
   hs_gram_key_clear(&s->gc_key);
   s->pre_y = s->pre_x = NULL;
   s->pre_valid = false;
   s->pre_scale = 1.0;
   s->regmask = NULL;
   s->trsv_epoch = 0;
   s->lan_sync = NULL;
   s->lan_rot[0] = s->lan_rot[1] = 0;
   s->last_status = HIPSDP_STATUS_UNSOLVED;
   s->sol_scale = 1.0;
   s->pc.on = getenv("HIPSDP_PHASES") != NULL && atoi(getenv("HIPSDP_PHASES")) != 0;
   s->pc.open = -1;
   for (int p = 0; p < PH_COUNT; ++p) s->pc.ms[p] = 0.0;
   s->stage_h[0] = s->stage_h[1] = s->stage_d[0] = s->stage_d[1] = NULL;
   s->stage_ev[0] = s->stage_ev[1] = NULL;
   s->stage_cap = 0;
   s->b = s->Dext = s->y = s->x = s->z = s->yt = s->dyt = s->wt = s->AX = s->AH = s->tmpe = s->rp = s->rd = s->tmpq = s->hl = NULL;
   s->beta = s->elp = s->dxa = s->dza = s->dx = s->dz = s->xs = s->zs = s->ys = s->u1 = s->rhs2 = s->cvec = s->u2 = s->dy = s->dya = NULL;
   s->Mx = s->Lm = s->dinvm = s->Slp = s->sc = s->red_ws = s->gemv_ws = s->lan_ws = s->lan_ws2 = NULL;
   s->gemvt_ws = NULL;
   s->gemvt_ws_len = 0;
   hipsdp_default_params(&s->par);
   s->sparse_policy = getenv("HIPSDP_SPARSE") != NULL ? atoi(getenv("HIPSDP_SPARSE")) : 1;
   if ( s->sparse_policy < 0 || s->sparse_policy > 2 ) s->sparse_policy = 1;
   if ( hipStreamCreateWithFlags(&s->stream, hipStreamNonBlocking) != hipSuccess
      || hipStreamCreateWithFlags(&s->stream2, hipStreamNonBlocking) != hipSuccess
      || hipEventCreateWithFlags(&s->evFork, hipEventDisableTiming) != hipSuccess
      || hipEventCreateWithFlags(&s->evJoin, hipEventDisableTiming) != hipSuccess
      || hipEventCreate(&s->ev0) != hipSuccess || hipEventCreate(&s->ev1) != hipSuccess )
   {
      delete s;
      set_err("stream/event creation failed");
      return HIPSDP_ERR_HIP;
   }
   (void) __sync_add_and_fetch(&g_live_solvers, 1);
   *out = s;
   return HIPSDP_OK;
}

static void master_free(hipsdp_solver* s)
{
   for (auto& B : s->blk)
      if ( B.sparse && B.sp_gathered && B.sp != NULL )
      {
         hs_sp_free(B.sp);
         B.sp = NULL;
      }
   for (double* p : s->master_A) if ( p != NULL ) dfree(p);
   for (hs_spm* M : s->master_sp) hs_spm_free(M);
   s->master_sp.clear();
   s->master_A.clear();
   s->master_sizes.clear();
   s->master_slots.clear();
   s->master_nvars = 0;
// ... 2570 lines not shown
{
   hipsdp_solver* s = static_cast<hipsdp_solver*>(arg);
   HS_CALL( fork2(s) );
   for (auto& B : s->blk)
      HS_CALL( hs_trtri(s->stream2, B.n, B.Lx, B.dinvx, B.LxInv, B.T1) );
   HS_HIP( hipEventRecord(s->evJoin, s->stream2) );
   s->sws.ev_g2 = (void*) s->evJoin;
   return HS_OK;
}

struct GeneralSolve
{
   hipsdp_solver* const s;
   hipsdp_info* const info;
   const std::chrono::steady_clock::time_point t_begin;
   const hipsdp_params& par = s->par;
   const hipStream_t st = s->stream;
   const int m = s->m, m1 = s->m + 1, q = s->q, K = (int) s->blk.size();
   const int settings = par.settings;
   const double gamma_eff = settings == 0 ? par.gamma : fmin(par.gamma, settings == 1 ? 0.9 : 0.75);
   const int stall_lim = settings == 0 ? 3 : (settings == 1 ? 5 : 8);
   const int nobest_lim = settings == 0 ? 6 : (settings == 1 ? 10 : 15);
   const double sigma_floor = settings == 0 ? 1e-8 : (settings == 1 ? 1e-4 : 1e-2);
   const bool no_identity_start = getenv("HIPSDP_NO_IDENTITY_START") != NULL && getenv("HIPSDP_NO_IDENTITY_START")[0] == '1';
   const bool optimistic = (s->comm == NULL) && getenv("HIPSDP_NO_OPTIMISTIC") == NULL;
   const char* const overstep = getenv("HIPSDP_TEST_OVERSTEP");

   double N1 = 0.0, normb = 0.0, normC = 0.0;
   bool small_all = false;
   int setf = 0;
   bool defer_ok = false;
   hipStream_t st2 = NULL;

   int it = 0, status = HIPSDP_STATUS_ITERLIM;
   bool stop = false;
   bool identity_start = false;
   bool factors_valid = false;
   bool residuals_ready = false;
   bool want_cert = false;
   bool rd_have = false;
   bool rd_pending = false;
   double rd_scale = 1.0;
   bool zchain_queued = false, xchain_queued = false;

   int certwait = 0, nstall = 0, sincebest = 0;
   double lastmu = 1e300, alpha_last = 1.0, bestmerit = 1e300;

   HostScalars hs;
   int hflags[3] = {0, 0, 0};
   double mu = 0, pinf = 0, dinf = 0, dabs = 0, gap = 0, pobj = 0, dobj = 0, rg = 0;
   double schur_ms = 0.0;
   bool defer_join = false, gram_only_used = false, schur_small = false;
   bool gram_cached = false;
   bool predH_queued = false, predH_joined = false, split_dz = false;
   double dta = 0, dka = 0, sigma = 0, eta = 0, amax = 0, alpha = 0, dt = 0, dk = 0;
   double tau0 = 0, kappa0 = 0, applied = 0;

   int halt(int why) { status = why; stop = true; return HS_OK; }

   int factor(hipStream_t qf, int n, double* L, double* dinv, const double* M, int f)
   {
      HS_CALL( hs_copy(qf, L, M, (long long) n * n) );
      return hs_potrf(qf, n, L, dinv, s->flags + f, NULL);
   }

   int z_chain(Block& B, hipStream_t qz)
   {
      const int n = B.n;
      if ( !factors_valid )
         HS_CALL( factor(qz, n, B.Lz, B.dinvz, B.Z, 0) );
      HS_CALL( hs_trtri(qz, n, B.Lz, B.dinvz, B.LzInv, B.T2) );
      HS_CALL( gemm_on(qz, HS_MC, HS_MC, n, n, n, 1.0, B.LzInv, n, B.LzInv, n, 0.0, B.Zinv, n, HS_GEMM_LOWER) );
      return hs_mirror_lower(qz, B.Zinv, n, n);
   }

   int x_chain(Block& B, bool inverse)
   {
      const int n = B.n;
      if ( !factors_valid )
         HS_CALL( factor(st, n, B.Lx, B.dinvx, B.X, 1) );
      HS_CALL( hs_zero_upper(st, B.Lx, n) );
      return inverse ? hs_trtri(st, n, B.Lx, B.dinvx, B.LxInv, B.T1) : HS_OK;
   }

   int queue_z_chains()
   {
      HS_CALL( fork2(s) );
      for (auto& B : s->blk)
         if ( B.n > 64 )
            HS_CALL( z_chain(B, st2) );
      zchain_queued = true;
      return HS_OK;
   }

   int read_back(int* flags3)
   {
      const std::function<int()> x_chains = [this]() -> int
      {
         for (auto& B : s->blk)
            if ( B.n > 64 )
               HS_CALL( x_chain(B, true) );
         xchain_queued = true;
         return HS_OK;
      };
      const bool with_x = zchain_queued && !xchain_queued && s->comm == NULL && !(factors_valid && defer_ok);
      return read_scalars(s, hs, flags3, with_x ? &x_chains : NULL);
   }

   void swap_trial()
   {
      for (auto& B : s->blk)
         if ( B.n <= 64 )
         {
            std::swap(B.X, B.Xs);
            std::swap(B.Z, B.Zs);
         }
   }

   int apply_step()
   {
      HS_CALL( hs_axpy3(st, alpha - applied, m, s->dy, s->y, q, s->dx, s->x, q, s->dz, s->z) );
      applied = alpha;
      s->tau = tau0 + alpha * dt;
      s->kappa = kappa0 + alpha * dk;
      return HS_OK;
   }

   int give_up(bool undo)
   {
      if ( par.verbose )
         printf("hipsdp: no step length down to %g keeps X and Z positive definite\n", alpha);
      if ( undo )
      {
         HS_CALL( hs_axpy3(st, -applied, m, s->dy, s->y, q, s->dx, s->x, q, s->dz, s->z) );
         s->tau = tau0;
         s->kappa = kappa0;
      }
      for (auto& B : s->blk)
      {
         B.derived_valid = false;
         if ( B.n <= 64 )
            continue;
         HS_CALL( hs_copy(st, B.X, B.Xs, (long long) B.n * B.n) );
         HS_CALL( hs_copy(st, B.Z, B.Zs, (long long) B.n * B.n) );
      }
      return halt(HIPSDP_STATUS_NUMERIC);
   }

   int start()
   {
      HS_CALL( stage_sync(s) );
      HS_CALL( ensure_schur_ws(s) );
      HS_CALL( ensure_packed(s) );
      int nmaxb = 0;
      long long N = q;
      small_all = (s->comm == NULL);
      for (auto& B : s->blk)
      {
         nmaxb = std::max(nmaxb, B.n);
// ... 283 lines not shown
      }
      if ( par.timelimit > 0.0 )
      {
         const double el = std::chrono::duration<double>(std::chrono::steady_clock::now() - t_begin).count();
         int over = el > par.timelimit ? 1 : 0;
         if ( s->comm != NULL )
         {
            HS_HIP( hipMemcpyAsync(s->flags + 7, &over, sizeof(int), hipMemcpyHostToDevice, st) );
            HS_CALL( hs_bcast_ints(s->comm, s->flags + 7, 1, st) );
            HS_HIP( hipMemcpyAsync(&over, s->flags + 7, sizeof(int), hipMemcpyDeviceToHost, st) );
            HS_HIP( hipStreamSynchronize(st) );
         }
         if ( over )
         {
            return halt(HIPSDP_STATUS_TIMELIM);
         }
      }
      return HS_OK;
   }

   int factorize()
   {
      phase_mark(s, PH_FACTOR);
      defer_join = defer_ok && !(identity_start && it == 0) && !xchain_queued;
      if ( !zchain_queued )
      {
         if ( !(setf && m <= 64) )
            HS_HIP( hipMemsetAsync(s->flags, 0, 8 * sizeof(int), st) );
         HS_CALL( fork2(s) );
      }
      for (auto& B : s->blk)
      {
         const int n = B.n;
         if ( n > 64 )
         {
            if ( !zchain_queued )
               HS_CALL( z_chain(B, st2) );
            if ( !xchain_queued )
               HS_CALL( x_chain(B, !defer_join) );
            continue;
         }
         if ( !(factors_valid && B.derived_valid) )
         {
            HS_CALL( hs_potrf_small_ext(st2, n, B.Lz, B.dinvz, s->flags + 0, B.Z, NULL, 0.0, NULL, B.LzInv, n <= 32 ? B.Zinv : NULL, setf) );
            HS_CALL( hs_potrf_small_ext(st, n, B.Lx, B.dinvx, s->flags + 1, B.X, NULL, 0.0, NULL, B.LxInv, NULL, setf) );
            B.derived_valid = true;
         }
         if ( n > 32 )
         {
            HS_CALL( gemm_on(st2, HS_MC, HS_MC, n, n, n, 1.0, B.LzInv, n, B.LzInv, n, 0.0, B.Zinv, n, HS_GEMM_LOWER) );
            HS_CALL( hs_mirror_lower(st2, B.Zinv, n, n) );
         }
      }
      zchain_queued = xchain_queued = false;
      if ( !defer_join )
         return join2(s);
      s->sws.after_g1 = after_g1_x_inverse;
      s->sws.after_g1_arg = s;
      return HS_OK;
   }

   int assemble()
   {
      phase_mark(s, PH_SCHUR);
      gram_only_used = gram_cached = false;
      hs_comm_phase(0);
      const bool clk_this = s->clk_on && s->clk_buf != NULL && s->clk_stream != NULL && s->clk_n < CLK_MAX_ASSEMBLIES;
      HS_HIP( hipEventRecord(s->ev0, st) );
      if ( clk_this )
      {
         HS_HIP( hipMemsetAsync(s->clk_buf + 4 * s->clk_n, 0, 4 * sizeof(unsigned long long), st) );
         HS_HIP( hipEventRecord(s->ev0, st) );
         HS_HIP( hipStreamWaitEvent(s->clk_stream, s->ev0, 0) );
         hipLaunchKernelGGL(k_clock_window, dim3(1), dim3(1), 0, s->clk_stream, s->clk_buf + 4 * s->clk_n);
         HS_LAUNCH_CHECK();
      }
      const double mfma_flops_before = hs_mfma_flops_total();
      schur_small = false;
      if ( s->comm == NULL && !s->shardA && !s->schur_mode_rows && !s->schur_mode_forced && K > 0 )
      {
         std::vector<int> bn;
         std::vector<const double*> bA, bX, bZ;
         bool anysp = false;
         for (auto& B : s->blk)
         {
            bn.push_back(B.n); bA.push_back(B.A); bX.push_back(B.X); bZ.push_back(B.Zinv);
            anysp = anysp || B.sparse;
         }
         const int rs = anysp ? 0 : hs_schur_small(st, m1, K, bn.data(), bA.data(), bX.data(), bZ.data(), q, s->Dext, s->x, s->z, s->Mx,
            m > 0 ? s->Lm : NULL, s->dya);
         if ( rs < 0 )
            return -rs;
         schur_small = (rs == 1);
      }
      if ( !schur_small )
         HS_CALL( assemble_forms() );
      if ( defer_join )
      {
         s->sws.ev_g2 = NULL;
         s->sws.after_g1 = NULL;
         HS_CALL( join2(s) );
      }
      HS_HIP( hipEventRecord(s->ev1, st) );
      if ( clk_this )
      {
         hipLaunchKernelGGL(k_clock_stop, dim3(1), dim3(1), 0, st, s->clk_buf + 4 * s->clk_n);
         HS_LAUNCH_CHECK();
         ++s->clk_n;
      }
      info->schur_flops_executed += hs_mfma_flops_total() - mfma_flops_before;
      hs_comm_phase(2);
      return HS_OK;
   }

   bool identity_packed(const Block& B) const
   {
      return B.Apk != NULL && hs_schur_identity_packed_fits(&s->sws, m1, B.n);
   }

   bool gram_cache_key(hs_gram_key* key)
   {
      if ( !(identity_start && it == 0) || s->comm != NULL || s->shardA || s->schur_mode_cols || s->schur_mode_rows || K < 1
         || K > HS_GRAM_MAXBLK )
         return false;
      int bn[HS_GRAM_MAXBLK], form[HS_GRAM_MAXBLK];
      unsigned long long gen[HS_GRAM_MAXBLK];
      for (int k = 0; k < K; ++k)
      {
         const Block& B = s->blk[k];
         if ( B.sparse || B.a_escaped )
            return false;
         bn[k] = B.n;
         form[k] = identity_packed(B) ? HS_GRAM_FORM_PACKED : HS_GRAM_FORM_FULL;
         gen[k] = B.A_gen;
      }
      if ( !hs_gram_key_make(key, m, K, bn, form, gen, s->sws.kws_len, s->sws.chunk_cols, s->sws.full) )
         return false;
      const long long len = (long long) (m1 + 32) * m1;
      if ( s->gc_M != NULL && s->gc_len != len )
      {
         (void) hipFree(s->gc_M);
         s->gc_M = NULL;
         s->gc_nomem = false;
         hs_gram_key_clear(&s->gc_key);
      }
      if ( s->gc_M == NULL && !s->gc_nomem )
      {
         if ( hipMalloc((void**) &s->gc_M, (size_t) len * sizeof(double)) != hipSuccess )
         {
            (void) hipGetLastError();
            s->gc_M = NULL;
            s->gc_nomem = true;
         }
         s->gc_len = len;
         hs_gram_key_clear(&s->gc_key);
      }
      return s->gc_M != NULL;
   }

   int assemble_forms()
   {
      hs_gram_key gkey;
      const bool gram_keyed = gram_cache_key(&gkey);
      gram_cached = gram_keyed && hs_gram_key_match(&s->gc_key, &gkey);
      if ( !gram_cached )
         HS_CALL( hs_fill(st, s->Mx, (long long) m1 * m1, 0.0) );
      if ( gram_cached )
      {
         HS_CALL( hs_copy(st, s->Mx, s->gc_M, s->gc_len) );
         ++s->gc_hits;
         gram_only_used = true;
      }
      else if ( s->shardA )
      {
         for (auto& B : s->blk)
            if ( !B.sparse )
               HS_CALL( hs_schur_Wvar_all(st, s->stream2, s->comm, s->rank, s->nranks, m1, B.n, B.A, B.Lx, B.LzInv, s->Mx, &s->sws, s->var_cw,
                     s->var_overlap ? 1 : 0) );
         HS_CALL( hs_allreduce_sum(s->comm, s->Mx, (long long) m1 * m1, st) );
      }
      else if ( s->schur_mode_cols )
      {
         const int S = s->schur_sim_shards;
         const int per = S / (s->comm != NULL ? s->nranks : 1);
         const int g0 = (s->comm != NULL ? s->rank : 0) * per;
         for (int g = g0; g < g0 + per; ++g)
            for (auto& B : s->blk)
            {
               if ( B.sparse )
                  continue;
               int c0, cw;
               hs_shard_cols(m1, B.n, S, g, &c0, &cw);
               if ( identity_start && it == 0 )
               {
                  if ( g == g0 )
                  {
                     const long long n2 = (long long) B.n * B.n;
                     const int G = s->comm != NULL ? s->nranks : 1, r = s->comm != NULL ? s->rank : 0;
                     const long long k0 = ((n2 * r / G) / 8) * 8, k1 = r == G - 1 ? n2 : ((n2 * (r + 1) / G) / 8) * 8;
                     HS_CALL( hs_schur_W_identity_range(st, m1, B.n, B.A, k0, k1, s->Mx, &s->sws) );
                  }
                  gram_only_used = true;
                  continue;
               }
               HS_CALL( hs_schur_Wcols(st, m1, B.n, B.A, B.Lx, B.LzInv, s->Mx, &s->sws, c0, cw) );
            }
         if ( s->comm != NULL )
            HS_CALL( hs_allreduce_sum(s->comm, s->Mx, (long long) m1 * m1, st) );
      }
      else if ( s->comm != NULL || s->schur_mode_rows )
      {
         int c, b1, b2;
         hs_shard_rows(m1, s->nranks, s->rank, &c, &b1, &b2);
         for (auto& B : s->blk)
         {
            if ( B.sparse )
               continue;
            HS_CALL( hs_schur_Urows(st, m1, B.n, B.A, B.X, B.Zinv, s->Mx, &s->sws, b1, b1 + c) );
            HS_CALL( hs_schur_Urows(st, m1, B.n, B.A, B.X, B.Zinv, s->Mx, &s->sws, b2, b2 + c) );
         }
         if ( s->comm != NULL )
         {
            const long long cnt = (long long) c * m1;
            HS_CALL( hs_allgather_inplace(s->comm, s->Mx, cnt, s->rank, st) );
            HS_CALL( hs_allgather(s->comm, s->Mx + (long long) b2 * m1, s->Mgather, cnt, st) );
            for (int r = 0; r < s->nranks; ++r)
            {
               const long long dstrow = (long long) (2 * s->nranks - 1 - r) * c;
               if ( dstrow >= m1 )
                  continue;
               long long rowsleft = m1 - dstrow;
               if ( rowsleft > c ) rowsleft = c;
               HS_CALL( hs_copy(st, s->Mx + dstrow * m1, s->Mgather + (long long) r * cnt, rowsleft * m1) );
            }
         }
         HS_CALL( hs_mirror_upper(st, s->Mx, m1, m1) );
      }
      else
      {
         for (auto& B : s->blk)
         {
            if ( B.sparse )
               continue;
            if ( identity_start && it == 0 )
            {
               assert(B.Apk == NULL || B.apk_valid);
               if ( identity_packed(B) )
                  HS_CALL( hs_schur_W_identity_packed(st, m1, B.n, B.Apk, B.Lp, s->Mx, &s->sws) );
               else
                  HS_CALL( hs_schur_W_identity(st, m1, B.n, B.A, s->Mx, &s->sws) );
               gram_only_used = true;
            }
            else if ( s->schur_mode_U )
               HS_CALL( hs_schur_U(st, m1, B.n, B.A, B.X, B.Zinv, s->Mx, &s->sws, 0, m1) );
            else
               HS_CALL( hs_schur_W(st, m1, B.n, B.A, B.Lx, B.LzInv, s->Mx, &s->sws) );
         }
         if ( gram_keyed )
         {
            ++s->gc_misses;
            HS_CALL( hs_copy(st, s->gc_M, s->Mx, s->gc_len) );
            s->gc_key = gkey;
         }
      }
      for (auto& B : s->blk)
      {
         if ( !B.sparse )
            continue;
         const int n = B.n;
         HS_CALL( gemm(s, HS_KC, HS_MC, n, n, n, 1.0, B.X, n, B.A0, n, 0.0, B.T1, n) );
         HS_CALL( gemm(s, HS_KC, HS_MC, n, n, n, 1.0, B.T1, n, B.Zinv, n, 0.0, B.W, n) );
         HS_CALL( pass_A(s, B, B.W, s->tmpe) );
         hipLaunchKernelGGL(k_add_col0, g1d(m1), dim3(256), 0, st, m1, s->tmpe, s->Mx);
         HS_LAUNCH_CHECK();
         HS_CALL( hs_sp_schur(st, B.sp, B.X, B.Zinv, s->Mx) );
      }
      if ( q > 0 )
      {
         HS_CALL( hs_lp_scale_rows(st, q, m1, s->x, s->z, s->Dext, s->Slp) );
         HS_CALL( gemm(s, HS_MC, HS_MC, m1, m1, q, 1.0, s->Dext, m1, s->Slp, m1, 1.0, s->Mx, m1, HS_GEMM_LOWER) );
      }
      return hs_mirror_lower(st, s->Mx, m1, m1);
   }

   int solve_m()
   {
      phase_mark(s, PH_MSOLVE);
      predH_queued = predH_joined = split_dz = false;
      if ( s->use2 && s->comm == NULL && !small_problem(s) && m > 0 )
      {
         HS_CALL( fork2(s) );
         {
            QueueSwap sw(s);
            HS_CALL( direction(s, 0.0, 1.0, mu, rg, false, 0.0, 1) );
         }
         predH_queued = true;
      }
      if ( m > 0 )
      {
         if ( !schur_small )
         {
            HS_HIP( hipMemcpy2DAsync(s->Lm, (size_t) m * sizeof(double), s->Mx + m1 + 1, (size_t) m1 * sizeof(double),
                  (size_t) m * sizeof(double), (size_t) m, hipMemcpyDeviceToDevice, st) );
            HS_HIP( hipMemcpy2DAsync(s->dya, sizeof(double), s->Mx + m1 + 1, (size_t) (m1 + 1) * sizeof(double), sizeof(double), (size_t) m,
                  hipMemcpyDeviceToDevice, st) );
         }
         HS_CALL( hs_potrf_psd(st, m, s->Lm, s->dinvm, s->flags + 2, s->dya, s->regmask, setf) );
         if ( m <= 64 )
         {
            HS_CALL( hs_solve2_small(st, m, s->Mx, s->b, s->dinvm, s->Lm, s->rhs2, s->u2, s->wt, hs_small_solve_by_substitution()) );
         }
         else
         {
            hipLaunchKernelGGL(k_rhs2, g1d(m), dim3(256), 0, st, m, s->Mx, s->b, s->rhs2);
            HS_LAUNCH_CHECK();
            if ( predH_queued )
            {
               HS_CALL( join2(s) );
               predH_joined = true;
               HS_CALL( hs_trsv_sync(st, m, s->Lm, s->dinvm, 3, s->rhs2, m, SOLVE_MODE, s->trsv_ws, &s->trsv_epoch) );
            }
            else
               HS_CALL( hs_trsv_sync(st, m, s->Lm, s->dinvm, 2, s->rhs2, m, SOLVE_MODE, s->trsv_ws, &s->trsv_epoch) );
         }
      }
      split_dz = predH_joined && s->comm == NULL;
      for (auto& B : s->blk)
         if ( B.Apk == NULL )
            split_dz = false;
      const bool tail = general_tail(s);
      if ( m == 0 || m > 64 )
         HS_CALL( hs_ipm_after_solve2(st, m, s->rhs2, s->u2, s->wt, s->u1, (split_dz && tail) ? s->cvec : NULL, s->cvec + m1, 1) );
      hs_red_batch_begin(st);
      HS_CALL( hs_fill_scalar(st, s->sc + SC_S0, 0.0) );
      if ( split_dz && !tail )
      {
         HS_CALL( hs_make_ext(st, m, 1.0, 1.0, s->u2, s->cvec) );
         HS_CALL( hs_make_ext(st, m, 0.0, 1.0, s->u1, s->cvec + m1) );
         HS_LAUNCH_CHECK();
      }
      int slot = 0;
      for (auto& B : s->blk)
      {
         const int n = B.n;
         const long long n2 = (long long) n * n;
         bool swept = false;
         if ( split_dz )
         {
            if ( B.P2 == NULL )
            {
               HS_CALL( dalloc(&B.P2, n2) );
               HS_CALL( dalloc(&B.pk3, 3 * B.Lp) );
            }
            const int r3 = hs_gemv_t3(st, m1, B.Lp, B.Apk, B.Lp, s->wt, s->cvec, s->cvec + m1, B.pk3, B.pk3 + B.Lp, B.pk3 + 2 * B.Lp);
            if ( r3 < 0 )
               return -r3;
            if ( r3 == 1 )
            {
               if ( tail )
               {
// ... 150 lines not shown
   {
      if ( it == 2 && overstep != NULL )
         alpha = amax * atof(overstep);
      for (int attempt = 0; attempt < 8; ++attempt)
      {
         HS_HIP( hipMemsetAsync(s->flags, 0, 8 * sizeof(int), st) );
         bool large = false, small = false;
         for (auto& B : s->blk)
            (B.n > 64 ? large : small) = true;
         if ( large && s->busy2 )
            HS_CALL( join2(s) );
         for (auto& B : s->blk)
         {
            if ( B.n <= 64 )
               continue;
            const hs_trial_job tj[2] = {{B.X, B.dX, B.Xs, B.Lx}, {B.Z, B.dZ, B.Zs, B.Lz}};
            HS_CALL( hs_trial_pair(st, (long long) B.n * B.n, alpha, attempt == 0 ? 1 : 0, tj) );
            const hs_potrf_job pj[2] = {{B.Lx, B.dinvx, s->flags + 1}, {B.Lz, B.dinvz, s->flags + 0}};
            HS_CALL( hs_potrf_pair(st, B.n, pj) );
         }
         if ( small )
         {
            HS_CALL( fork2(s) );
            for (auto& B : s->blk)
            {
               const int n = B.n;
               if ( n > 64 )
                  continue;
               HS_CALL( hs_potrf_small_ext(st, n, B.Lx, B.dinvx, s->flags + 1, B.X, B.dX, alpha, B.Xs, B.LxInv, NULL, setf) );
               HS_CALL( hs_potrf_small_ext(st2, n, B.Lz, B.dinvz, s->flags + 0, B.Z, B.dZ, alpha, B.Zs, B.LzInv, n <= 32 ? B.Zinv : NULL, setf) );
            }
            HS_CALL( join2(s) );
         }
         if ( K == 0 )
            break;
         if ( optimistic )
         {
            swap_trial();
            HS_CALL( apply_step() );
            factors_valid = true;
            if ( s->use2 && !zchain_queued )
               HS_CALL( queue_z_chains() );
            if ( attempt == 0 )
            {
               rd_have = !small_problem(s);
               rd_pending = rd_have;
               rd_scale = 1.0 - alpha * eta;
            }
            HS_CALL( enqueue_residuals() );
            HS_CALL( read_back(hflags) );
            if ( hflags[0] == 0 && hflags[1] == 0 )
               break;
            swap_trial();
            factors_valid = zchain_queued = xchain_queued = false;
            rd_have = rd_pending = false;
         }
         else
         {
            if ( s->comm == NULL )
               HS_CALL( publish_and_wait(s, s->nsc, 2) );
            else
            {
               HS_CALL( hs_bcast_ints(s->comm, s->flags, 3, st) );
               HS_HIP( hipMemcpyAsync(s->hsc + s->nsc, s->flags, 4 * sizeof(int), hipMemcpyDeviceToHost, st) );
               HS_HIP( hipStreamSynchronize(st) );
            }
            memcpy(hflags, s->hsc + s->nsc, 3 * sizeof(int));
            if ( hflags[0] == 0 && hflags[1] == 0 )
               break;
         }
         alpha *= 0.5;
         info->chol_fail++;
      }
      if ( K > 0 && (hflags[0] != 0 || hflags[1] != 0) )
         return give_up(optimistic && applied != 0.0);
      if ( !optimistic )
         swap_trial();
      for (auto& B : s->blk)
         if ( B.n <= 64 )
            B.derived_valid = true;
      factors_valid = (K > 0);
      alpha_last = alpha;
      if ( optimistic && K > 0 )
      {
         residuals_ready = true;
         return HS_OK;
      }
      HS_CALL( hs_axpy3(st, alpha, m, s->dy, s->y, q, s->dx, s->x, q, s->dz, s->z) );
      s->tau += alpha * dt;
      s->kappa += alpha * dk;
      rd_have = !small_problem(s);
      rd_pending = rd_have;
      rd_scale = 1.0 - alpha * eta;
      return HS_OK;
   }

   int run()
   {
      HS_CALL( start() );
      for (it = 0; it <= par.maxiter; ++it)
      {
         if ( !residuals_ready )
            HS_CALL( residual_pass() );
         residuals_ready = false;
         HS_CALL( terminate() );
         if ( stop )
            break;
// ... 675 lines not shown
               const double* hy = pp[j].host + pp[j].hy;
               for (int i = 0; i < m; ++i)
                  Y[(size_t) J * m + i] = hy[i] * sol.sol_scale;
            }
         }
         if ( !chunk_ok )
         {
            (void) hipStreamSynchronize(st);
            for (int j = c0 + n; j < count; ++j) rc[j] = HIPSDP_ERR_HIP;
            all_published = false;
            break;
         }
         s->stage_off = so;
      }
      if ( all_published )
         s->stage_off = 0;
      if ( !all_published )
         later.clear();
   }

   double* home = L.dev;
   for (int J : later)
      rc[J] = objs_general_job(s, params, B + (size_t) J * m, home, off, warm, &infos[J], Y != NULL ? Y + (size_t) J * m : NULL);
   r = HIPSDP_OK;
   if ( !later.empty() )
      r = objs_home_copy(s, home, off, false, false, true);
   s->have_start = false;
   s->solved = false;
   s->s1_last = 0;
   s->s1_sol_host = false;
   return leave(solve_end(s, r));
}

extern "C" int hipsdp_solve_objectives_stats(long long* calls, long long* launches, long long* problems)
{
   if ( calls != NULL )
      *calls = __sync_add_and_fetch(&g_objs_calls, 0);
   if ( launches != NULL )
      *launches = __sync_add_and_fetch(&g_objs_launches, 0);
   if ( problems != NULL )
      *problems = __sync_add_and_fetch(&g_objs_problems, 0);
   return HIPSDP_OK;
}

extern "C" int hipsdp_gram_cache_stats(hipsdp_solver* s, long long* hits, long long* misses)
{
   if ( s == NULL )
      return HIPSDP_ERR_ARG;
   if ( hits != NULL ) *hits = s->gc_hits;
   if ( misses != NULL ) *misses = s->gc_misses;
   return HIPSDP_OK;
}

extern "C" int hipsdp_solve_many_stats(long long* launches, long long* problems)
{
   if ( launches != NULL )
      *launches = __sync_add_and_fetch(&g_many_launches, 0);
   if ( problems != NULL )
      *problems = __sync_add_and_fetch(&g_many_problems, 0);
   return HIPSDP_OK;
}

extern "C" long long hipsdp_solve1_fallbacks(void)
{
   return __sync_add_and_fetch(&g_solve1_fallbacks, 0);
}

extern "C" long long hipsdp_solve1_fallbacks_warm(void)
{
   return __sync_add_and_fetch(&g_solve1_fallbacks_warm, 0);
}

extern "C" long long hipsdp_solve1_solves(void)
{
   return __sync_add_and_fetch(&g_solve1_solves, 0);
}

extern "C" int hipsdp_solve1_debug_counts(unsigned int* counts2)
{
   if ( counts2 == NULL )
      return 0;
   return hs_solve1_debug_counts(counts2);
}

extern "C" int hipsdp_solve_path(hipsdp_solver* s)
{
   return (s != NULL && s->solved) ? s->s1_last : 0;
}

extern "C" int hipsdp_solve1_trace(hipsdp_solver* s, double* out64, int maxrows, double* hist)
{
   if ( s == NULL || s->s1_host == NULL )
      return HIPSDP_ERR_ARG;
   if ( out64 != NULL )
      memcpy(out64, s->s1_host, HS_S1_OUT_DOUBLES * sizeof(double));
   if ( hist != NULL && maxrows > 0 )
      memcpy(hist, s->s1_host + HS_S1_OUT_DOUBLES + 8, (size_t) (maxrows < S1_HIST_MAX ? maxrows : S1_HIST_MAX) * 16 * sizeof(double));
   return HIPSDP_OK;
}


static int read_scaled(hipsdp_solver* s, const double* d, long long n, double scale, double* out)
{
   if ( n <= 0 ) return HIPSDP_OK;
   if ( s->s1_sol_host && s->s1_host != NULL && (d == s->y || d == s->x || d == s->z) )
   {
// ... 489 lines not shown
```

scip-sdp_amd/csrc/schur.hip:

```cpp
#include "hs_kernels.h"
#include "hs_lds_product.h"
#include <vector>
#include <cmath>
#include <stdlib.h>

int hs_schur_ws_alloc(hs_schur_ws* w, int m1, long long n2max, double budget_gb)
{
   w->T = w->U = w->K = w->V = w->U2 = w->V2 = NULL;
   w->evP[0] = w->evP[1] = w->evX[0] = w->evX[1] = NULL;
   w->ev_g2 = NULL;
   w->after_g1 = NULL; w->after_g1_arg = NULL;
   w->capT = w->capV = 0;
   const double need_full = 2.0 * 8.0 * (double) m1 * (double) n2max;
   long long cols = m1;
   w->full = 1;
   if ( need_full > budget_gb * 1e9 )
   {
      w->full = 0;
      cols = (long long) (budget_gb * 1e9 / (2.0 * 8.0 * (double) n2max));
      cols = (cols / 128) * 128;
      if ( cols < 128 ) cols = 128;
      if ( cols > m1 ) cols = m1;
   }
   w->chunk_cols = cols;
// ... 107 lines not shown

int hs_schur_W_identity_range(hipStream_t s, int m1, int n, const double* A, long long k0, long long k1, double* Mx, hs_schur_ws* w)
{
   const long long n2 = (long long) n * n;
   const long long K = k1 - k0;
   if ( n2 > 2000000000LL || k0 < 0 || k1 > n2 || (k0 & 1) )
      return HS_ERR_ARG;
   if ( K <= 0 )
      return HS_OK;
   {
      int done = 0;
      HS_CALL( schur_gram(s, m1, K, A + k0, n2, Mx, w, &done) );
      if ( done )
         return HS_OK;
   }
   int flags, sk;
   schur_syrk_shape(w, m1, K, m1 >= SYRK_MIN_M1 && K >= 16384 && (K >= 50000 || m1 >= 900), &flags, &sk);
   hs_gemm_args g3 = {m1, m1, (int) K, HS_KC, HS_KC, A + k0, n2, 0, A + k0, n2, 0, Mx, m1, 0, 1.0, 1.0, 1, flags, sk, sk > 1 ? w->K : NULL};
   return hs_dgemm(s, &g3);
}

int hs_schur_W_identity(hipStream_t s, int m1, int n, const double* A, double* Mx, hs_schur_ws* w)
{
   return hs_schur_W_identity_range(s, m1, n, A, 0, (long long) n * n, Mx, w);
}

int hs_schur_identity_packed_fits(const hs_schur_ws* w, int m1, int n)
{
   return w->T != NULL && (long long) m1 * ((n + 1) & ~1) <= w->chunk_cols * w->n2;
}

int hs_schur_W_identity_packed(hipStream_t s, int m1, int n, const double* Apk, long long Lp, double* Mx, hs_schur_ws* w)
{
   const int ldd = (n + 1) & ~1;
   if ( n < 1 || Lp < (long long) n * (n + 1) / 2 || (Lp & 1) || Lp > 2000000000LL || !hs_schur_identity_packed_fits(w, m1, n) )
      return HS_ERR_ARG;
   int done = 0;
   HS_CALL( schur_gram(s, m1, Lp, Apk, Lp, Mx, w, &done, 2.0) );
   if ( !done )
   {
      int flags, sk;
      schur_syrk_shape(w, m1, Lp, m1 >= SYRK_MIN_M1 && Lp >= 16384 && (Lp >= 50000 || m1 >= 900), &flags, &sk);
      hs_gemm_args g3 = {m1, m1, (int) Lp, HS_KC, HS_KC, Apk, Lp, 0, Apk, Lp, 0, Mx, m1, 0, 2.0, 1.0, 1, flags, sk, sk > 1 ? w->K : NULL};
      HS_CALL( hs_dgemm(s, &g3) );
   }
   HS_CALL( hs_packed_diag(s, m1, n, ldd, Lp, Apk, w->T) );
   const bool slab = w->K != NULL && (long long) m1 * m1 <= w->kws_len;
   hs_gemm_args gd = {m1, m1, n, HS_KC, HS_KC, w->T, ldd, 0, w->T, ldd, 0, slab ? w->K : Mx, m1, 0, slab ? 1.0 : -1.0, slab ? 0.0 : 1.0, 1,
      HS_GEMM_LOWER, 1, NULL};
   HS_CALL( hs_dgemm(s, &gd) );
   return slab ? hs_sub_lower(s, m1, w->K, Mx) : HS_OK;
}

int hs_schur_W(hipStream_t s, int m1, int n, const double* A, const double* R, const double* G, double* Mx, hs_schur_ws* w)
{
   const long long n2 = (long long) n * n;
   const long long rows = (long long) m1 * n;
   if ( !w->full || n2 > 2000000000LL || rows > 2000000000LL )
      return HS_ERR_ARG;
   hs_gemm_args g1 = {(int) rows, n, n, HS_KC, HS_MC, A, n, 0, R, n, 0, w->T, n, 0, 1.0, 0.0, 1, HS_GEMM_B_LOWTRI, 1, NULL};
   HS_CALL( hs_dgemm(s, &g1) );
   if ( w->after_g1 != NULL )
   {
      int (*f)(void*) = w->after_g1;
      w->after_g1 = NULL;
      HS_CALL( f(w->after_g1_arg) );
   }
   if ( w->ev_g2 != NULL )
      HS_HIP( hipStreamWaitEvent(s, (hipEvent_t) w->ev_g2, 0) );
   hs_gemm_args g2 = {n, n, n, HS_KC, HS_MC, G, n, 0, w->T, n, n2, w->U, n, n2, 1.0, 0.0, m1, HS_GEMM_A_LOWTRI | HS_GEMM_REMAP, 1, NULL};
   HS_CALL( hs_dgemm(s, &g2) );
   {
      int done = 0;
      HS_CALL( schur_gram(s, m1, n2, w->U, n2, Mx, w, &done) );
      if ( done )
         return HS_OK;
   }
   int flags = HS_GEMM_LOWER;
   int sk;
   if ( m1 >= SYRK_MIN_M1 && n2 >= 16384 && (n2 >= 50000 || m1 >= 900) )
   {
      const long long tm = (m1 + 127) / 128;
      const long long ntri = tm * (tm + 1) / 2;
      sk = hs_dgemm_pick_xcd_slices(ntri, n2);
      while ( sk > 2 && (long long) sk * m1 * m1 > w->kws_len ) --sk;
      flags |= HS_GEMM_XCD;
      flags |= HS_GEMM_NOFAST;
   }
   else
   {
      sk = hs_dgemm_pick_splitk(m1, m1, (int) n2, 1);
      while ( sk > 1 && (long long) sk * m1 * m1 > w->kws_len ) --sk;
   }
   hs_gemm_args g3 = {m1, m1, (int) n2, HS_KC, HS_KC, w->U, n2, 0, w->U, n2, 0, Mx, m1, 0, 1.0, 1.0, 1, flags, sk, w->K};
   HS_CALL( hs_dgemm(s, &g3) );
   return HS_OK;
}

int hs_schur_Wcols(hipStream_t s, int m1, int n, const double* A, const double* R, const double* G, double* Mx, hs_schur_ws* w,
   int c0, int cw)
{
   if ( cw <= 0 )
      return HS_OK;
   const long long rows = (long long) m1 * n;
   const long long nk = (long long) n * cw;
   if ( c0 < 0 || c0 + cw > n || rows > 2000000000LL || nk > 2000000000LL || (long long) m1 * nk > w->chunk_cols * w->n2 )
      return HS_ERR_ARG;
   const int narrow = cw <= 64 ? HS_GEMM_TILE64 : 0;
   hs_gemm_args g1 = {(int) rows, cw, n - c0, HS_KC, HS_MC, A + c0, n, 0, R + (long long) c0 * n + c0, n, 0, w->T, cw, 0, 1.0, 0.0, 1,
      HS_GEMM_B_LOWTRI | narrow, 1, NULL};
   HS_CALL( hs_dgemm(s, &g1) );
   hs_gemm_args g2 = {n, cw, n, HS_KC, HS_MC, G, n, 0, w->T, cw, nk, w->U, cw, nk, 1.0, 0.0, m1, HS_GEMM_A_LOWTRI | HS_GEMM_REMAP | narrow, 1, NULL};
   HS_CALL( hs_dgemm(s, &g2) );
   {
      int done = 0;
      HS_CALL( schur_gram(s, m1, nk, w->U, nk, Mx, w, &done) );
      if ( done )
         return HS_OK;
   }
   int flags, sk;
   schur_syrk_shape(w, m1, nk, m1 >= 256 && nk >= 16384, &flags, &sk);
   hs_gemm_args g3 = {m1, m1, (int) nk, HS_KC, HS_KC, w->U, nk, 0, w->U, nk, 0, Mx, m1, 0, 1.0, 1.0, 1, flags, sk, sk > 1 ? w->K : NULL};
   HS_CALL( hs_dgemm(s, &g3) );
   return HS_OK;
// ... 412 lines not shown
```

scip-sdp_amd/csrc/units.hip:

```cpp
#include "hs_kernels.h"
#include "hs_gram_cache.h"
#include "../../include/hipsdp.h"
#include "../../include/hipsdp_units.h"
#include <vector>
#include <algorithm>
#include <cstring>
#include <cstdlib>

namespace {

struct DevBuf
{
   double* p;
   DevBuf() : p(NULL) {}
   ~DevBuf() { if ( p ) (void) hipFree(p); }
   int alloc(long long n) { if ( n <= 0 ) n = 1; hipError_t e = hipMalloc((void**) &p, (size_t) n * sizeof(double)); if ( e != hipSuccess ) { hs_record_hip_error(e, "hipMalloc", __FILE__, __LINE__); return e == hipErrorOutOfMemory ? HS_ERR_NOMEM : HS_ERR_HIP; } return HS_OK; }
   int up(const double* h, long long n) { if ( n <= 0 ) return HS_OK; hipError_t e = hipMemcpy(p, h, (size_t) n * sizeof(double), hipMemcpyHostToDevice); if ( e != hipSuccess ) { hs_record_hip_error(e, "H2D", __FILE__, __LINE__); return HS_ERR_HIP; } return HS_OK; }
   int down(double* h, long long n) { if ( n <= 0 ) return HS_OK; hipError_t e = hipMemcpy(h, p, (size_t) n * sizeof(double), hipMemcpyDeviceToHost); if ( e != hipSuccess ) { hs_record_hip_error(e, "D2H", __FILE__, __LINE__); return HS_ERR_HIP; } return HS_OK; }
};

int pick_device(int device)
{
   int nd = 0;
   if ( hipGetDeviceCount(&nd) != hipSuccess || nd <= 0 )
// ... 2120 lines not shown
   int t = 0, rc = HS_OK;
   if ( fused )
   {
      t = hs_gemv_t3(0, R, E, dA.p, lda, dc.p, dc.p + R, dc.p + 2LL * R, dO.p, dO.p + Ep, dO.p + 2 * Ep);
      if ( t < 0 ) { rc = -t; t = 0; }
   }
   if ( t == 0 )
      for (int v = 0; v < 3 && rc == HS_OK; ++v)
         rc = hs_gemv_t(0, R, E, dA.p, lda, dc.p + (long long) v * R, 0.0, NULL, dO.p + v * Ep);
   if ( hipDeviceSynchronize() != hipSuccess && rc == HS_OK ) rc = HS_ERR_HIP;
   HS_CALL( rc );
   if ( took != NULL ) *took = t;
   for (int v = 0; v < 3; ++v)
      HS_HIP( hipMemcpy(out + v * E, dO.p + v * Ep, (size_t) E * sizeof(double), hipMemcpyDeviceToHost) );
   return HIPSDP_OK;
}

extern "C" int hipsdp_pass_a_unit(int device, int R, long long E, long long lda, const double* A, int nv, const double* V, int voff,
   long long wsdoubles, double* out, int* info)
{
   if ( R < 1 || E < 1 || lda < E || A == NULL || nv < 1 || nv > 4 || V == NULL || voff < 0 || voff > 64 || wsdoubles < 0 || out == NULL )
      return HIPSDP_ERR_ARG;
   HS_CALL( pick_device(device) );
   const long long na = span(R, (int) E, lda), Ep = E + (E & 1);
   DevBuf dA, dV, dO, dW;
   HS_CALL( dA.alloc(na) ); HS_CALL( dV.alloc(nv * Ep + voff) ); HS_CALL( dO.alloc((long long) nv * R) ); HS_CALL( dW.alloc(wsdoubles) );
   HS_CALL( nan_fill(dO, (long long) nv * R) ); HS_CALL( nan_fill(dW, wsdoubles) );
   HS_CALL( dA.up(A, na) );
   const double* vp[4];
   for (int v = 0; v < nv; ++v)
   {
      HS_HIP( hipMemcpy(dV.p + voff + v * Ep, V + v * E, (size_t) E * sizeof(double), hipMemcpyHostToDevice) );
      vp[v] = dV.p + voff + v * Ep;
   }
   if ( info != NULL )
   {
      const bool vec = (lda & 1) == 0 && (voff & 1) == 0;
      long long nsplit = 1;
      if ( R < 512 && E >= 16384 )
      {
         nsplit = (1024 + R - 1) / R;
         if ( nsplit > E / 8192 ) nsplit = E / 8192;
         if ( nsplit < 1 ) nsplit = 1;
         if ( nsplit * nv * R > wsdoubles ) nsplit = 1;
      }
      info[0] = (int) nsplit; info[1] = vec ? 1 : 0;
   }
   hs_red_batch_reset();
   int rc = hs_gemv_n(0, R, E, dA.p, lda, nv, vp, dO.p, R, dW.p, wsdoubles);
   if ( hipDeviceSynchronize() != hipSuccess && rc == HS_OK ) rc = HS_ERR_HIP;
   HS_CALL( rc );
   return dO.down(out, (long long) nv * R);
}
```

Measured before the change: 13.66.

## Fuse Gram reduction with mirror and factor staging, cache Cholesky factors by Gram key

Adds a fused Gram-reduce kernel that writes the full symmetric Schur matrix plus the Lm copy and diagonal in one pass. This replaces the separate fill, reduce, mirror and two 2D copies before the PSD Cholesky. It also adds a factor store keyed on the Gram key and pivot parameters, so a repeated Schur matrix can reuse its Cholesky factor, and it skips redundant memsets of the GEMM counters. These cut launches and memory traffic, at the cost of extra device storage and cache-key correctness risk.

```diff
diff --git a/include/hipsdp.h b/include/hipsdp.h
--- a/include/hipsdp.h
+++ b/include/hipsdp.h
@@ -103,6 +103,7 @@
 
 HIPSDP_API int  hipsdp_solve(hipsdp_solver* solver, const hipsdp_params* params, hipsdp_info* info);
 HIPSDP_API int  hipsdp_gram_cache_stats(hipsdp_solver* solver, long long* hits, long long* misses);
+HIPSDP_API int  hipsdp_factor_store_stats(hipsdp_solver* solver, long long* hits, long long* misses);
 
 HIPSDP_API int  hipsdp_solve_path(hipsdp_solver* solver);
 HIPSDP_API long long hipsdp_solve1_solves(void);
diff --git a/include/hipsdp_units.h b/include/hipsdp_units.h
--- a/include/hipsdp_units.h
+++ b/include/hipsdp_units.h
@@ -106,6 +106,10 @@
    int* took);
 HIPSDP_API int  hipsdp_pass_a_unit(int device, int R, long long E, long long lda, const double* A, int nv, const double* V, int voff,
    long long wsdoubles, double* out, int* info);
+HIPSDP_API int  hipsdp_gram_to_factor_unit(int device, int M, int no, int nd, int nslab, const double* ws, int fused, double* Mx, double* Lm,
+   double* dya);
+HIPSDP_API int  hipsdp_schur_w_staged_unit(int device, int m1, int n, const double* A, const double* P, const double* Q, int staged,
+   double* Mx, double* Lm, double* dya, int* stages, int* used);
 
 #ifdef __cplusplus
 }
diff --git a/scip-sdp_amd/binding.py b/scip-sdp_amd/binding.py
--- a/scip-sdp_amd/binding.py
+++ b/scip-sdp_amd/binding.py
@@ -278,6 +278,12 @@
         hits = C.c_longlong(0)
         misses = C.c_longlong(0)
         _chk(self._l().hipsdp_gram_cache_stats(self.h, C.byref(hits), C.byref(misses)), "hipsdp_gram_cache_stats")
+        return hits.value, misses.value
+
+    def factor_store_stats(self):
+        hits = C.c_longlong(0)
+        misses = C.c_longlong(0)
+        _chk(self._l().hipsdp_factor_store_stats(self.h, C.byref(hits), C.byref(misses)), "hipsdp_factor_store_stats")
         return hits.value, misses.value
 
     def solve1_trace(self, rows=0):
@@ -900,6 +906,20 @@
     return Mx, tuple(used)
 
 
+def schur_w_staged_unit(A, R, G, staged, device=0):
+    A = _f64(A)
+    m1, n = A.shape[0], A.shape[1]
+    R = _f64(R); G = _f64(G)
+    assert m1 >= 2 and A.shape == (m1, n, n) and R.shape == (n, n) and G.shape == (n, n)
+    Mx, Lm, dya = np.zeros((m1, m1)), np.zeros((m1 - 1, m1 - 1)), np.zeros(m1 - 1)
+    used, stages = (C.c_int * 3)(0, 0, 0), C.c_int(-1)
+    _chk(ulib().hipsdp_schur_w_staged_unit(device, m1, n, _dp(A), _dp(R), _dp(G), int(staged), _dp(Mx), _dp(Lm), _dp(dya), C.byref(stages),
+                                           used), "hipsdp_schur_w_staged_unit")
+    if staged and not stages.value:
+        return None, None, None, 0, tuple(used)
+    return Mx, Lm, dya, stages.value, tuple(used)
+
+
 def schur_small_unit(As, Xs, Zinvs, Dext=None, x=None, z=None, fill=0.0, device=0):
     As = [_f64(a) for a in As]; Xs = [_f64(a) for a in Xs]; Zinvs = [_f64(a) for a in Zinvs]
     nblk, m1 = len(As), As[0].shape[0]
@@ -1242,6 +1262,16 @@
     return out, took.value
 
 
+def gram_to_factor_unit(ws, no, nd, fused, device=0):
+    ws = _f64(ws)
+    nslab, M, M2 = ws.shape
+    assert M == M2
+    Mx, Lm, dya = np.zeros((M, M)), np.zeros((M - 1, M - 1)), np.zeros(M - 1)
+    _chk(ulib().hipsdp_gram_to_factor_unit(device, M, int(no), int(nd), nslab, _dp(ws), int(fused), _dp(Mx), _dp(Lm), _dp(dya)),
+         "hipsdp_gram_to_factor_unit")
+    return Mx, Lm, dya
+
+
 def pass_a_unit(A, E, V, voff=0, wsdoubles=0, device=0):
     A, V = _f64(A), _f64(V)
     R, lda = A.shape
diff --git a/scip-sdp_amd/csrc/chol.hip b/scip-sdp_amd/csrc/chol.hip
--- a/scip-sdp_amd/csrc/chol.hip
+++ b/scip-sdp_amd/csrc/chol.hip
@@ -42,6 +42,7 @@
 
 #define PD_LD (NB + 2)
 #define PD_SMEM_BYTES ((2 * NB * PD_LD + 5 * NB) * (int) sizeof(double))
+#define PD_REGTOL 1e-13
 
 struct pd_ext
 {
@@ -725,7 +726,7 @@
    const int nS = nblk - kb;
    const int t = nblk - kb - 1;
    const int nT = kb > 0 ? t * (t + 1) / 2 : 0;
-   hipLaunchKernelGGL((k_potrf_step<NBK>), dim3(nS + nT), dim3(256), PD_SMEM_BYTES, s, A, lda, n, kb, nblk, dinv, flag, diag0, 1e-13, ext);
+   hipLaunchKernelGGL((k_potrf_step<NBK>), dim3(nS + nT), dim3(256), PD_SMEM_BYTES, s, A, lda, n, kb, nblk, dinv, flag, diag0, PD_REGTOL, ext);
    HS_LAUNCH_CHECK();
    return HS_OK;
 }
@@ -739,7 +740,7 @@
       ext = *extp;
    static hs_attr_mask attr_done;
    HS_CALL( hs_func_max_lds(reinterpret_cast<const void*>(&k_potrf_diag<NBK>), PD_SMEM_BYTES, &attr_done) );
-   hipLaunchKernelGGL((k_potrf_diag<NBK>), dim3(1), dim3(256), PD_SMEM_BYTES, s, Ajj, lda, nb, j0, dj, flag, diag0, 1e-13, ext);
+   hipLaunchKernelGGL((k_potrf_diag<NBK>), dim3(1), dim3(256), PD_SMEM_BYTES, s, Ajj, lda, nb, j0, dj, flag, diag0, PD_REGTOL, ext);
    HS_LAUNCH_CHECK();
    return HS_OK;
 }
@@ -844,13 +845,26 @@
    return HS_OK;
 }
 
+static int potrf_pivot_rule()
+{
+   static int rule = getenv("HIPSDP_PIVOT_RULE") != NULL ? atoi(getenv("HIPSDP_PIVOT_RULE")) : 3;
+   return rule;
+}
+
+void hs_potrf_psd_params(int* rule, double* regtol, int* variant)
+{
+   *rule = potrf_pivot_rule();
+   *regtol = PD_REGTOL;
+   *variant = g_potrf_force_v1 ? 1 : 0;
+}
+
 int hs_potrf_psd(hipStream_t s, int n, double* A, double* dinv, int* flag, const double* diag0, int* regmask, int set_flag)
 {
    if ( n <= 0 )
       return HS_OK;
    if ( diag0 != NULL && regmask == NULL && n > NB )
       return HS_ERR_ARG;
-   static int rule = getenv("HIPSDP_PIVOT_RULE") != NULL ? atoi(getenv("HIPSDP_PIVOT_RULE")) : 3;
+   const int rule = potrf_pivot_rule();
    pd_ext ext = {NULL, NULL, 0.0, NULL, NULL, NULL, (set_flag && n <= NB) ? 1 : 0, rule, regmask};
    const pd_ext* extp = ((diag0 != NULL && regmask != NULL) || ext.set_flag) ? &ext : NULL;
    const long long lda = n;
diff --git a/scip-sdp_amd/csrc/dgemm2.hip b/scip-sdp_amd/csrc/dgemm2.hip
--- a/scip-sdp_amd/csrc/dgemm2.hip
+++ b/scip-sdp_amd/csrc/dgemm2.hip
@@ -1241,22 +1241,41 @@
    return g5_wide_mode >= 0;
 }
 
-static unsigned int* g5_counters(hipStream_t stream)
+struct g5_ctr
+{
+   unsigned int* p;
+   bool cleared;
+};
+
+static g5_ctr* g5_counters(hipStream_t stream)
 {
    static std::mutex mu;
-   static std::map<std::pair<int, hipStream_t>, unsigned int*> tab;
+   static std::map<std::pair<int, hipStream_t>, g5_ctr> tab;
    int dev = 0;
    if ( hipGetDevice(&dev) != hipSuccess )
       return NULL;
    std::lock_guard<std::mutex> lk(mu);
    auto it = tab.find(std::make_pair(dev, stream));
    if ( it != tab.end() )
-      return it->second;
+      return &it->second;
    unsigned int* q = NULL;
    if ( hipMalloc((void**) &q, 64) != hipSuccess )
       return NULL;
-   tab[std::make_pair(dev, stream)] = q;
-   return q;
+   const g5_ctr c = {q, false};
+   return &(tab[std::make_pair(dev, stream)] = c);
+}
+
+int hs_dgemm5_preclear(hipStream_t stream)
+{
+   g5_ctr* c = g5_counters(stream);
+   if ( c == NULL )
+      return HS_ERR_HIP;
+   if ( c->cleared )
+      return HS_OK;
+   if ( hipMemsetAsync(c->p, 0, 64, stream) != hipSuccess )
+      return HS_ERR_HIP;
+   c->cleared = true;
+   return HS_OK;
 }
 
 int hs_dgemm2_tri5_eligible(const hs_gemm_args* a)
@@ -1334,9 +1353,11 @@
       }
       if ( hs_func_max_lds(fn5, (int) smem5, &attr5[inst5]) != HS_OK )
          return -HS_ERR_HIP;
-      unsigned int* ctr = g5_counters(stream);
-      if ( ctr == NULL || hipMemsetAsync(ctr, 0, 64, stream) != hipSuccess )
+      g5_ctr* const c5 = g5_counters(stream);
+      if ( c5 == NULL || (!c5->cleared && hipMemsetAsync(c5->p, 0, 64, stream) != hipSuccess) )
          return -HS_ERR_HIP;
+      c5->cleared = false;
+      unsigned int* const ctr = c5->p;
       hs_gemm_args a5 = *a;
       a5.flags |= G5_F_NT | G5_F_SETS | G5_F_PAIRS;
       const long long tm5 = triB && wide ? (a->M + 2 * G2_BT - 1) / (2 * G2_BT) : tm;
diff --git a/scip-sdp_amd/csrc/gram.hip b/scip-sdp_amd/csrc/gram.hip
--- a/scip-sdp_amd/csrc/gram.hip
+++ b/scip-sdp_amd/csrc/gram.hip
@@ -339,6 +339,68 @@
       double* q = C + (long long) r * ldc + c;
       *q = beta != 0.0 ? alpha * s + beta * (*q) : alpha * s;
    }
+}
+
+#define GR_RT 32
+__global__ void __launch_bounds__(256) hs_gram_reduce_fused_kernel(int M, int no, int nd, const double* __restrict__ ws,
+   double* __restrict__ C, long long ldc, double alpha, double* __restrict__ Lm, double* __restrict__ dya)
+{
+   __shared__ double t[GR_RT][GR_RT + 1];
+   const int tr = blockIdx.y, tc = blockIdx.x;
+   if ( tc > tr )
+      return;
+   const long long MM = (long long) M * M;
+   const long long ldl = M - 1;
+   const int r0 = tr * GR_RT, c0 = tc * GR_RT;
+   const int ns = (r0 / GR_BT == c0 / GR_BT) ? nd : no;
+   const int lc = threadIdx.x & (GR_RT - 1), l0 = threadIdx.x / GR_RT;
+   for (int lr = l0; lr < GR_RT; lr += 256 / GR_RT)
+   {
+      const int r = r0 + lr, c = c0 + lc;
+      if ( r < M && c <= r )
+      {
+         const long long e = (long long) r * M + c;
+         double sum = 0.0;
+#pragma unroll 4
+         for (int k = 0; k < ns; ++k)
+            sum += ws[(long long) k * MM + e];
+         const double v = alpha * sum;
+         t[lr][lc] = v;
+         C[(long long) r * ldc + c] = v;
+         if ( Lm != NULL && c >= 1 )
+            Lm[(long long) (r - 1) * ldl + (c - 1)] = v;
+         if ( dya != NULL && r == c && r >= 1 )
+            dya[r - 1] = v;
+      }
+   }
+   __syncthreads();
+   for (int lr = l0; lr < GR_RT; lr += 256 / GR_RT)
+   {
+      const int r = c0 + lr, c = r0 + lc;
+      if ( c < M && r < c )
+      {
+         const double v = t[lc][lr];
+         C[(long long) r * ldc + c] = v;
+         if ( Lm != NULL && r >= 1 )
+            Lm[(long long) (r - 1) * ldl + (c - 1)] = v;
+      }
+   }
+}
+
+int hs_gram_reduce(hipStream_t stream, int M, int no, int nd, const double* ws, double* C, long long ldc, double alpha, double beta)
+{
+   int blocks = (int) (((long long) M * M + 255) / 256);
+   if ( blocks > 2048 ) blocks = 2048;
+   hipLaunchKernelGGL(hs_gram_reduce_kernel, dim3(blocks), dim3(256), 0, stream, M, no, nd, ws, C, ldc, alpha, beta);
+   return hipGetLastError() != hipSuccess ? HS_ERR_HIP : HS_OK;
+}
+
+int hs_gram_reduce_fused(hipStream_t stream, int M, int no, int nd, const double* ws, double* C, long long ldc, double alpha, double* Lm,
+   double* dya)
+{
+   const int T = (M + GR_RT - 1) / GR_RT;
+   hipLaunchKernelGGL(hs_gram_reduce_fused_kernel, dim3(T, T), dim3(256), 0, stream, M, no, nd, ws, C, ldc, alpha, Lm, dya);
+   return hipGetLastError() != hipSuccess ? HS_ERR_HIP : HS_OK;
 }
 
 namespace {
@@ -505,16 +567,29 @@
    return __atomic_load_n(&gr_taken, __ATOMIC_RELAXED);
 }
 
-int hs_gram_try(hipStream_t stream, int M, long long K, const double* W, long long ldw, double* C, long long ldc, double alpha, double beta,
-   double* ws, int nslab, double* executed)
+static GramPlan* gr_eligible(int M, long long K, const double* W, long long ldw, const double* ws, int nslab)
 {
    if ( ws == NULL || nslab < 2 || M < 256 || K < 16384 )
-      return 0;
+      return NULL;
    if ( (ldw & 1) || (K & 1) || (((uintptr_t) W) & 15) || K > 2000000000LL )
-      return 0;
+      return NULL;
    if ( nslab > 64 ) nslab = 64;
    GramPlan* P = gr_plan(M, K, nslab);
    if ( P == NULL || P->dev == NULL || P->items.size() < 256 )
+      return NULL;
+   return P;
+}
+
+int hs_gram_takes(int M, long long K, const double* W, long long ldw, const double* ws, int nslab)
+{
+   return gr_eligible(M, K, W, ldw, ws, nslab) != NULL ? 1 : 0;
+}
+
+static int gr_try(hipStream_t stream, int M, long long K, const double* W, long long ldw, double* C, long long ldc, double alpha, double beta,
+   double* ws, int nslab, double* executed, bool fused, double* Lm, double* dya)
+{
+   GramPlan* P = gr_eligible(M, K, W, ldw, ws, nslab);
+   if ( P == NULL )
       return 0;
    gram_args g;
    g.W = W; g.ldw = ldw; g.M = M; g.ws = ws; g.items = P->dev; g.off = P->devoff;
@@ -525,17 +600,25 @@
    hipLaunchKernelGGL(hs_gram_kernel, dim3(512), dim3(256), smem, stream, g);
    if ( hipGetLastError() != hipSuccess )
       return -HS_ERR_HIP;
-   {
-      int blocks = (int) (((long long) M * M + 255) / 256);
-      if ( blocks > 2048 ) blocks = 2048;
-      hipLaunchKernelGGL(hs_gram_reduce_kernel, dim3(blocks), dim3(256), 0, stream, M, P->no, P->nd, ws, C, ldc, alpha, beta);
-      if ( hipGetLastError() != hipSuccess )
-         return -HS_ERR_HIP;
-   }
+   if ( (fused ? hs_gram_reduce_fused(stream, M, P->no, P->nd, ws, C, ldc, alpha, Lm, dya)
+               : hs_gram_reduce(stream, M, P->no, P->nd, ws, C, ldc, alpha, beta)) != HS_OK )
+      return -HS_ERR_HIP;
    if ( executed != NULL )
       *executed = P->executed;
    (void) __atomic_add_fetch(&gr_taken, 1, __ATOMIC_RELAXED);
    return 1;
+}
+
+int hs_gram_try(hipStream_t stream, int M, long long K, const double* W, long long ldw, double* C, long long ldc, double alpha, double beta,
+   double* ws, int nslab, double* executed)
+{
+   return gr_try(stream, M, K, W, ldw, C, ldc, alpha, beta, ws, nslab, executed, false, NULL, NULL);
+}
+
+int hs_gram_try_fused(hipStream_t stream, int M, long long K, const double* W, long long ldw, double* C, long long ldc, double alpha,
+   double* ws, int nslab, double* executed, double* Lm, double* dya)
+{
+   return gr_try(stream, M, K, W, ldw, C, ldc, alpha, 0.0, ws, nslab, executed, true, Lm, dya);
 }
 
 int hs_gram_plan_info(int M, long long K, int nslab, int* no, int* nd, int* nitems, double* span)
diff --git a/scip-sdp_amd/csrc/hs_common.h b/scip-sdp_amd/csrc/hs_common.h
--- a/scip-sdp_amd/csrc/hs_common.h
+++ b/scip-sdp_amd/csrc/hs_common.h
@@ -86,6 +86,7 @@
 int hs_dgemm(hipStream_t stream, const hs_gemm_args* args);
 int hs_dgemm2_try(hipStream_t stream, const hs_gemm_args* args, int kchunk);
 int hs_dgemm2_enable(int on);
+int hs_dgemm5_preclear(hipStream_t stream);
 int hs_dgemm2_paired_taken(void);
 int hs_dgemm2_wide_force(int mode);
 int hs_dgemm2_tri5_forced(void);
@@ -93,6 +94,12 @@
 
 int hs_gram_try(hipStream_t stream, int M, long long K, const double* W, long long ldw, double* C, long long ldc, double alpha, double beta,
    double* ws, int nslab, double* executed);
+int hs_gram_takes(int M, long long K, const double* W, long long ldw, const double* ws, int nslab);
+int hs_gram_try_fused(hipStream_t stream, int M, long long K, const double* W, long long ldw, double* C, long long ldc, double alpha,
+   double* ws, int nslab, double* executed, double* Lm, double* dya);
+int hs_gram_reduce(hipStream_t stream, int M, int no, int nd, const double* ws, double* C, long long ldc, double alpha, double beta);
+int hs_gram_reduce_fused(hipStream_t stream, int M, int no, int nd, const double* ws, double* C, long long ldc, double alpha, double* Lm,
+   double* dya);
 int hs_gram_plan_info(int M, long long K, int nslab, int* no, int* nd, int* nitems, double* span);
 
 int hs_dgemm3_try(hipStream_t stream, const hs_gemm_args* args);
diff --git a/scip-sdp_amd/csrc/hs_gram_cache.h b/scip-sdp_amd/csrc/hs_gram_cache.h
--- a/scip-sdp_amd/csrc/hs_gram_cache.h
+++ b/scip-sdp_amd/csrc/hs_gram_cache.h
@@ -64,4 +64,59 @@
    return 1;
 }
 
+struct hs_factor_key
+{
+   int valid;
+   hs_gram_key gram;
+   int rule, set_flag, variant;
+   double regtol;
+   long long dinv_len;
+};
+
+static inline void hs_factor_key_clear(hs_factor_key* k)
+{
+   k->valid = 0;
+   hs_gram_key_clear(&k->gram);
+   k->rule = k->set_flag = k->variant = 0;
+   k->regtol = 0.0;
+   k->dinv_len = 0;
+}
+
+struct hs_factor_case
+{
+   int gram_keyed;
+   int q;
+   int one_launch;
+};
+
+static inline int hs_factor_key_make(hs_factor_key* k, const hs_factor_case* c, const hs_gram_key* gram, int rule, double regtol,
+   int set_flag, int variant, long long dinv_len)
+{
+   hs_factor_key_clear(k);
+   if ( !c->gram_keyed || c->q != 0 || c->one_launch || !gram || !gram->valid || gram->m < 1 || dinv_len < 1 || !(regtol == regtol) )
+      return 0;
+   k->gram = *gram;
+   k->rule = rule;
+   k->regtol = regtol;
+   k->set_flag = set_flag ? 1 : 0;
+   k->variant = variant;
+   k->dinv_len = dinv_len;
+   k->valid = 1;
+   return 1;
+}
+
+static inline int hs_factor_key_match(const hs_factor_key* have, const hs_factor_key* want)
+{
+   return have->valid && want->valid && have->rule == want->rule && have->regtol == want->regtol && have->set_flag == want->set_flag
+      && have->variant == want->variant && have->dinv_len == want->dinv_len && hs_gram_key_match(&have->gram, &want->gram);
+}
+
+static inline long long hs_factor_off_dinv(int m) { return (long long) m * m; }
+static inline long long hs_factor_off_dya(int m, long long dinv_len) { return hs_factor_off_dinv(m) + dinv_len; }
+static inline long long hs_factor_off_ints(int m, long long dinv_len) { return hs_factor_off_dya(m, dinv_len) + m; }
+static inline long long hs_factor_store_len(int m, long long dinv_len)
+{
+   return hs_factor_off_ints(m, dinv_len) + ((long long) m + 1 + 1) / 2;
+}
+
 #endif
diff --git a/scip-sdp_amd/csrc/hs_kernels.h b/scip-sdp_amd/csrc/hs_kernels.h
--- a/scip-sdp_amd/csrc/hs_kernels.h
+++ b/scip-sdp_amd/csrc/hs_kernels.h
@@ -105,6 +105,9 @@
 int  hs_schur_U(hipStream_t s, int m1, int n, const double* A, const double* X, const double* Zinv, double* Mx,
    hs_schur_ws* w, int j_begin, int j_end);
 int  hs_schur_W(hipStream_t s, int m1, int n, const double* A, const double* R, const double* G, double* Mx, hs_schur_ws* w);
+int  hs_schur_W_stages(const hs_schur_ws* w, int m1, int n);
+int  hs_schur_W_staged(hipStream_t s, int m1, int n, const double* A, const double* R, const double* G, double* Mx, hs_schur_ws* w, double* Lm,
+   double* dya);
 int  hs_schur_W_identity(hipStream_t s, int m1, int n, const double* A, double* Mx, hs_schur_ws* w);
 int  hs_schur_W_identity_range(hipStream_t s, int m1, int n, const double* A, long long k0, long long k1, double* Mx, hs_schur_ws* w);
 int  hs_schur_W_identity_packed(hipStream_t s, int m1, int n, const double* Apk, long long Lp, double* Mx, hs_schur_ws* w);
@@ -189,6 +192,7 @@
 int hs_potrf(hipStream_t s, int n, double* A, double* dinv, int* flag, const double* diag0);
 long long hs_potrf_dinv_len(int n);
 int hs_potrf_psd(hipStream_t s, int n, double* A, double* dinv, int* flag, const double* diag0, int* regmask, int set_flag);
+void hs_potrf_psd_params(int* rule, double* regtol, int* variant);
 struct hs_potrf_job { double* A; double* dinv; int* flag; };
 int hs_potrf_pair(hipStream_t s, int n, const hs_potrf_job* jobs);
 int hs_trtri(hipStream_t s, int n, const double* L, const double* dinv, double* Linv, double* tmp);
diff --git a/scip-sdp_amd/csrc/ipm.hip b/scip-sdp_amd/csrc/ipm.hip
--- a/scip-sdp_amd/csrc/ipm.hip
+++ b/scip-sdp_amd/csrc/ipm.hip
@@ -244,7 +244,17 @@
    double* gc_M; long long gc_len; bool gc_nomem;
    hs_gram_key gc_key;
    long long gc_hits, gc_misses;
+   double* fs_buf; long long fs_len; bool fs_nomem;
+   hs_factor_key fs_key;
+   long long fs_hits, fs_misses;
 };
+
+static void factor_store_free(hipsdp_solver* s)
+{
+   if ( s->fs_buf != NULL ) (void) hipFree(s->fs_buf);
+   s->fs_buf = NULL; s->fs_len = 0; s->fs_nomem = false;
+   hs_factor_key_clear(&s->fs_key);
+}
 
 static void a_written(hipsdp_solver* s, Block& B)
 {
@@ -519,6 +529,7 @@
    if ( s->gc_M != NULL ) (void) hipFree(s->gc_M);
    s->gc_M = NULL; s->gc_len = 0; s->gc_nomem = false;
    hs_gram_key_clear(&s->gc_key);
+   factor_store_free(s);
    if ( s->ln_dev != NULL ) (void) hipFree(s->ln_dev);
    if ( s->ln_host != NULL ) (void) hipHostFree(s->ln_host);
    s->ln_dev = NULL; s->ln_host = NULL; s->ln_host_dev = NULL; s->ln_dev_len = 0; s->ln_host_len = 0;
@@ -588,6 +599,8 @@
    s->trsv_ws = NULL;
    s->a_gen_next = 0; s->gc_M = NULL; s->gc_len = 0; s->gc_nomem = false; s->gc_hits = s->gc_misses = 0;
    hs_gram_key_clear(&s->gc_key);
+   s->fs_buf = NULL; s->fs_len = 0; s->fs_nomem = false; s->fs_hits = s->fs_misses = 0;
+   hs_factor_key_clear(&s->fs_key);
    s->pre_y = s->pre_x = NULL;
    s->pre_valid = false;
    s->pre_scale = 1.0;
@@ -3264,6 +3277,10 @@
    double schur_ms = 0.0;
    bool defer_join = false, gram_only_used = false, schur_small = false;
    bool gram_cached = false;
+   bool gram_keyed_cur = false;
+   hs_gram_key gkey_cur;
+   bool lm_staged = false;
+   bool xzero_queued = false;
    bool predH_queued = false, predH_joined = false, split_dz = false;
    double dta = 0, dka = 0, sigma = 0, eta = 0, amax = 0, alpha = 0, dt = 0, dk = 0;
    double tau0 = 0, kappa0 = 0, applied = 0;
@@ -3291,7 +3308,8 @@
       const int n = B.n;
       if ( !factors_valid )
          HS_CALL( factor(st, n, B.Lx, B.dinvx, B.X, 1) );
-      HS_CALL( hs_zero_upper(st, B.Lx, n) );
+      if ( !factors_valid || !xzero_queued )
+         HS_CALL( hs_zero_upper(st, B.Lx, n) );
       return inverse ? hs_trtri(st, n, B.Lx, B.dinvx, B.LxInv, B.T1) : HS_OK;
    }
 
@@ -3316,7 +3334,15 @@
          return HS_OK;
       };
       const bool with_x = zchain_queued && !xchain_queued && s->comm == NULL && !(factors_valid && defer_ok);
-      return read_scalars(s, hs, flags3, with_x ? &x_chains : NULL);
+      const std::function<int()> ahead = [this]() -> int
+      {
+         for (auto& B : s->blk)
+            HS_CALL( hs_zero_upper(st, B.Lx, B.n) );
+         xzero_queued = true;
+         return hs_dgemm5_preclear(st);
+      };
+      const bool with_ahead = !with_x && zchain_queued && !xchain_queued && !xzero_queued && s->comm == NULL && factors_valid && defer_ok;
+      return read_scalars(s, hs, flags3, with_x ? &x_chains : (with_ahead ? &ahead : NULL));
    }
 
    void swap_trial()
@@ -3706,7 +3732,7 @@
             HS_CALL( hs_mirror_lower(st2, B.Zinv, n, n) );
          }
       }
-      zchain_queued = xchain_queued = false;
+      zchain_queued = xchain_queued = xzero_queued = false;
       if ( !defer_join )
          return join2(s);
       s->sws.after_g1 = after_g1_x_inverse;
@@ -3717,7 +3743,7 @@
    int assemble()
    {
       phase_mark(s, PH_SCHUR);
-      gram_only_used = gram_cached = false;
+      gram_only_used = gram_cached = gram_keyed_cur = lm_staged = false;
       hs_comm_phase(0);
       const bool clk_this = s->clk_on && s->clk_buf != NULL && s->clk_stream != NULL && s->clk_n < CLK_MAX_ASSEMBLIES;
       HS_HIP( hipEventRecord(s->ev0, st) );
@@ -3797,6 +3823,7 @@
          s->gc_M = NULL;
          s->gc_nomem = false;
          hs_gram_key_clear(&s->gc_key);
+         factor_store_free(s);
       }
       if ( s->gc_M == NULL && !s->gc_nomem )
       {
@@ -3812,12 +3839,54 @@
       return s->gc_M != NULL;
    }
 
+   bool factor_store_key(hs_factor_key* key)
+   {
+      const hs_factor_case fc = {gram_keyed_cur ? 1 : 0, q, schur_small ? 1 : 0};
+      int rule, variant;
+      double regtol;
+      hs_potrf_psd_params(&rule, &regtol, &variant);
+      const long long nd = hs_potrf_dinv_len(m);
+      if ( !hs_factor_key_make(key, &fc, &gkey_cur, rule, regtol, setf, variant, nd) )
+         return false;
+      const long long len = hs_factor_store_len(m, nd);
+      if ( s->fs_buf != NULL && s->fs_len != len )
+         factor_store_free(s);
+      if ( s->fs_buf == NULL && !s->fs_nomem )
+      {
+         if ( hipMalloc((void**) &s->fs_buf, (size_t) len * sizeof(double)) != hipSuccess )
+         {
+            (void) hipGetLastError();
+            s->fs_buf = NULL;
+            s->fs_nomem = true;
+         }
+         s->fs_len = len;
+         hs_factor_key_clear(&s->fs_key);
+      }
+      return s->fs_buf != NULL;
+   }
+
+   int factor_store_move(bool store)
+   {
+      const long long nd = hs_potrf_dinv_len(m);
+      double* const part[3] = {s->fs_buf, s->fs_buf + hs_factor_off_dinv(m), s->fs_buf + hs_factor_off_dya(m, nd)};
+      double* const live[3] = {s->Lm, s->dinvm, s->dya};
+      const long long cnt[3] = {(long long) m * m, nd, m};
+      for (int k = 0; k < 3; ++k)
+         HS_CALL( hs_copy(st, store ? part[k] : live[k], store ? live[k] : part[k], cnt[k]) );
+      int* const ints = reinterpret_cast<int*>(s->fs_buf + hs_factor_off_ints(m, nd));
+      HS_HIP( hipMemcpyAsync(store ? ints : s->regmask, store ? s->regmask : ints, (size_t) m * sizeof(int), hipMemcpyDeviceToDevice, st) );
+      HS_HIP( hipMemcpyAsync(store ? ints + m : s->flags + 2, store ? s->flags + 2 : ints + m, sizeof(int), hipMemcpyDeviceToDevice, st) );
+      return HS_OK;
+   }
+
    int assemble_forms()
    {
-      hs_gram_key gkey;
-      const bool gram_keyed = gram_cache_key(&gkey);
+      hs_gram_key& gkey = gkey_cur;
+      const bool gram_keyed = gram_keyed_cur = gram_cache_key(&gkey);
       gram_cached = gram_keyed && hs_gram_key_match(&s->gc_key, &gkey);
-      if ( !gram_cached )
+      const bool staged = !(identity_start && it == 0) && s->comm == NULL && !s->shardA && !s->schur_mode_cols && !s->schur_mode_rows
+         && !s->schur_mode_U && K == 1 && !s->blk[0].sparse && q == 0 && m > 0 && hs_schur_W_stages(&s->sws, m1, s->blk[0].n);
+      if ( !gram_cached && !staged )
          HS_CALL( hs_fill(st, s->Mx, (long long) m1 * m1, 0.0) );
       if ( gram_cached )
       {
@@ -3907,6 +3976,12 @@
             }
             else if ( s->schur_mode_U )
                HS_CALL( hs_schur_U(st, m1, B.n, B.A, B.X, B.Zinv, s->Mx, &s->sws, 0, m1) );
+            else if ( staged )
+            {
+               HS_CALL( hs_schur_W_staged(st, m1, B.n, B.A, B.Lx, B.LzInv, s->Mx, &s->sws, s->Lm, s->dya) );
+               lm_staged = true;
+               return HS_OK;
+            }
             else
                HS_CALL( hs_schur_W(st, m1, B.n, B.A, B.Lx, B.LzInv, s->Mx, &s->sws) );
          }
@@ -3952,14 +4027,30 @@
       }
       if ( m > 0 )
       {
-         if ( !schur_small )
-         {
-            HS_HIP( hipMemcpy2DAsync(s->Lm, (size_t) m * sizeof(double), s->Mx + m1 + 1, (size_t) m1 * sizeof(double),
-                  (size_t) m * sizeof(double), (size_t) m, hipMemcpyDeviceToDevice, st) );
-            HS_HIP( hipMemcpy2DAsync(s->dya, sizeof(double), s->Mx + m1 + 1, (size_t) (m1 + 1) * sizeof(double), sizeof(double), (size_t) m,
-                  hipMemcpyDeviceToDevice, st) );
-         }
-         HS_CALL( hs_potrf_psd(st, m, s->Lm, s->dinvm, s->flags + 2, s->dya, s->regmask, setf) );
+         hs_factor_key fkey;
+         const bool factor_keyed = factor_store_key(&fkey);
+         if ( factor_keyed && hs_factor_key_match(&s->fs_key, &fkey) )
+         {
+            HS_CALL( factor_store_move(false) );
+            ++s->fs_hits;
+         }
+         else
+         {
+            if ( !schur_small && !lm_staged )
+            {
+               HS_HIP( hipMemcpy2DAsync(s->Lm, (size_t) m * sizeof(double), s->Mx + m1 + 1, (size_t) m1 * sizeof(double),
+                     (size_t) m * sizeof(double), (size_t) m, hipMemcpyDeviceToDevice, st) );
+               HS_HIP( hipMemcpy2DAsync(s->dya, sizeof(double), s->Mx + m1 + 1, (size_t) (m1 + 1) * sizeof(double), sizeof(double), (size_t) m,
+                     hipMemcpyDeviceToDevice, st) );
+            }
+            HS_CALL( hs_potrf_psd(st, m, s->Lm, s->dinvm, s->flags + 2, s->dya, s->regmask, setf) );
+            if ( factor_keyed )
+            {
+               HS_CALL( factor_store_move(true) );
+               s->fs_key = fkey;
+               ++s->fs_misses;
+            }
+         }
          if ( m <= 64 )
          {
             HS_CALL( hs_solve2_small(st, m, s->Mx, s->b, s->dinvm, s->Lm, s->rhs2, s->u2, s->wt, hs_small_solve_by_substitution()) );
@@ -4216,7 +4307,7 @@
             if ( hflags[0] == 0 && hflags[1] == 0 )
                break;
             swap_trial();
-            factors_valid = zchain_queued = xchain_queued = false;
+            factors_valid = zchain_queued = xchain_queued = xzero_queued = false;
             rd_have = rd_pending = false;
          }
          else
@@ -4998,6 +5089,15 @@
    return HIPSDP_OK;
 }
 
+extern "C" int hipsdp_factor_store_stats(hipsdp_solver* s, long long* hits, long long* misses)
+{
+   if ( s == NULL )
+      return HIPSDP_ERR_ARG;
+   if ( hits != NULL ) *hits = s->fs_hits;
+   if ( misses != NULL ) *misses = s->fs_misses;
+   return HIPSDP_OK;
+}
+
 extern "C" int hipsdp_solve_many_stats(long long* launches, long long* problems)
 {
    if ( launches != NULL )
diff --git a/scip-sdp_amd/csrc/schur.hip b/scip-sdp_amd/csrc/schur.hip
--- a/scip-sdp_amd/csrc/schur.hip
+++ b/scip-sdp_amd/csrc/schur.hip
@@ -183,7 +183,37 @@
    return slab ? hs_sub_lower(s, m1, w->K, Mx) : HS_OK;
 }
 
+static long long schur_gram_slabs(const hs_schur_ws* w, int m1)
+{
+   const long long nslab = w->kws_len / ((long long) m1 * m1);
+   return nslab > 64 ? 64 : nslab;
+}
+
+int hs_schur_W_stages(const hs_schur_ws* w, int m1, int n)
+{
+   const long long n2 = (long long) n * n;
+   return w->full && n2 <= 2000000000LL && (long long) m1 * n <= 2000000000LL
+      && hs_gram_takes(m1, n2, w->U, n2, w->K, (int) schur_gram_slabs(w, m1));
+}
+
+static int schur_W(hipStream_t s, int m1, int n, const double* A, const double* R, const double* G, double* Mx, hs_schur_ws* w, bool staged,
+   double* Lm, double* dya);
+
 int hs_schur_W(hipStream_t s, int m1, int n, const double* A, const double* R, const double* G, double* Mx, hs_schur_ws* w)
+{
+   return schur_W(s, m1, n, A, R, G, Mx, w, false, NULL, NULL);
+}
+
+int hs_schur_W_staged(hipStream_t s, int m1, int n, const double* A, const double* R, const double* G, double* Mx, hs_schur_ws* w, double* Lm,
+   double* dya)
+{
+   if ( !hs_schur_W_stages(w, m1, n) )
+      return HS_ERR_ARG;
+   return schur_W(s, m1, n, A, R, G, Mx, w, true, Lm, dya);
+}
+
+static int schur_W(hipStream_t s, int m1, int n, const double* A, const double* R, const double* G, double* Mx, hs_schur_ws* w, bool staged,
+   double* Lm, double* dya)
 {
    const long long n2 = (long long) n * n;
    const long long rows = (long long) m1 * n;
@@ -201,6 +231,17 @@
       HS_HIP( hipStreamWaitEvent(s, (hipEvent_t) w->ev_g2, 0) );
    hs_gemm_args g2 = {n, n, n, HS_KC, HS_MC, G, n, 0, w->T, n, n2, w->U, n, n2, 1.0, 0.0, m1, HS_GEMM_A_LOWTRI | HS_GEMM_REMAP, 1, NULL};
    HS_CALL( hs_dgemm(s, &g2) );
+   if ( staged )
+   {
+      double executed = 0.0;
+      const int r = hs_gram_try_fused(s, m1, n2, w->U, n2, Mx, m1, 1.0, w->K, (int) schur_gram_slabs(w, m1), &executed, Lm, dya);
+      if ( r < 0 )
+         return -r;
+      if ( r != 1 )
+         return HS_ERR_ARG;
+      hs_mfma_flops_add(executed);
+      return HS_OK;
+   }
    {
       int done = 0;
       HS_CALL( schur_gram(s, m1, n2, w->U, n2, Mx, w, &done) );
diff --git a/scip-sdp_amd/csrc/units.hip b/scip-sdp_amd/csrc/units.hip
--- a/scip-sdp_amd/csrc/units.hip
+++ b/scip-sdp_amd/csrc/units.hip
@@ -2196,3 +2196,84 @@
    HS_CALL( rc );
    return dO.down(out, (long long) nv * R);
 }
+
+extern "C" int hipsdp_gram_to_factor_unit(int device, int M, int no, int nd, int nslab, const double* ws, int fused, double* Mx, double* Lm,
+   double* dya)
+{
+   if ( M < 2 || M > 4096 || nslab < 1 || nslab > 64 || no < 1 || no > nslab || nd < 1 || nd > nslab || ws == NULL || !flag01(fused)
+         || Mx == NULL || Lm == NULL || dya == NULL )
+      return HIPSDP_ERR_ARG;
+   HS_CALL( pick_device(device) );
+   const int m = M - 1;
+   const long long MM = (long long) M * M, mm = (long long) m * m;
+   DevBuf dW, dM, dL, dG;
+   HS_CALL( dW.alloc(nslab * MM) ); HS_CALL( dM.alloc(MM) ); HS_CALL( dL.alloc(mm) ); HS_CALL( dG.alloc(m) );
+   HS_CALL( nan_fill(dM, MM) ); HS_CALL( nan_fill(dL, mm) ); HS_CALL( nan_fill(dG, m) );
+   HS_CALL( dW.up(ws, nslab * MM) );
+   hs_red_batch_reset();
+   int rc = HS_OK;
+   if ( fused )
+      rc = hs_gram_reduce_fused(0, M, no, nd, dW.p, dM.p, M, 1.0, dL.p, dG.p);
+   else
+   {
+      rc = hs_fill(0, dM.p, MM, 0.0);
+      if ( rc == HS_OK ) rc = hs_gram_reduce(0, M, no, nd, dW.p, dM.p, M, 1.0, 1.0);
+      if ( rc == HS_OK ) rc = hs_mirror_lower(0, dM.p, M, M);
+      if ( rc == HS_OK && hipMemcpy2DAsync(dL.p, (size_t) m * sizeof(double), dM.p + M + 1, (size_t) M * sizeof(double), (size_t) m * sizeof(double),
+               (size_t) m, hipMemcpyDeviceToDevice, 0) != hipSuccess ) rc = HS_ERR_HIP;
+      if ( rc == HS_OK && hipMemcpy2DAsync(dG.p, sizeof(double), dM.p + M + 1, (size_t) (M + 1) * sizeof(double), sizeof(double), (size_t) m,
+               hipMemcpyDeviceToDevice, 0) != hipSuccess ) rc = HS_ERR_HIP;
+   }
+   if ( hipDeviceSynchronize() != hipSuccess && rc == HS_OK ) rc = HS_ERR_HIP;
+   HS_CALL( rc );
+   HS_CALL( dM.down(Mx, MM) ); HS_CALL( dL.down(Lm, mm) );
+   return dG.down(dya, m);
+}
+
+extern "C" int hipsdp_schur_w_staged_unit(int device, int m1, int n, const double* A, const double* P, const double* Q, int staged,
+   double* Mx, double* Lm, double* dya, int* stages, int* used)
+{
+   HS_CALL( pick_device(device) );
+   if ( m1 < 2 || n < 1 || A == NULL || P == NULL || Q == NULL || !flag01(staged) || Mx == NULL || Lm == NULL || dya == NULL || stages == NULL )
+      return HIPSDP_ERR_ARG;
+   const long long n2 = (long long) n * n, MM = (long long) m1 * m1;
+   const int m = m1 - 1;
+   if ( n2 > 2000000000LL || (long long) m1 * n > 2000000000LL || MM > 2000000000LL )
+      return HIPSDP_ERR_ARG;
+   DevBuf dA, dP, dQ, dM, dL, dG;
+   HS_CALL( dA.alloc(m1 * n2) ); HS_CALL( dP.alloc(n2) ); HS_CALL( dQ.alloc(n2) ); HS_CALL( dM.alloc(MM) );
+   HS_CALL( dL.alloc((long long) m * m) ); HS_CALL( dG.alloc(m) );
+   HS_CALL( dA.up(A, m1 * n2) ); HS_CALL( dP.up(P, n2) ); HS_CALL( dQ.up(Q, n2) );
+   HS_CALL( nan_fill(dM, MM) ); HS_CALL( nan_fill(dL, (long long) m * m) ); HS_CALL( nan_fill(dG, m) );
+   hs_schur_ws w;
+   int rc = hs_schur_ws_alloc(&w, m1, n2, 40.0);
+   if ( rc != HS_OK )
+      return rc;
+   const int t2 = hs_dgemm2_enable(1), t5 = hs_dgemm2_paired_taken(), tg = hs_gram_taken();
+   *stages = hs_schur_W_stages(&w, m1, n);
+   if ( staged && *stages )
+      rc = hs_schur_W_staged(0, m1, n, dA.p, dP.p, dQ.p, dM.p, &w, dL.p, dG.p);
+   else if ( !staged )
+   {
+      rc = hs_fill(0, dM.p, MM, 0.0);
+      if ( rc == HS_OK ) rc = hs_schur_W(0, m1, n, dA.p, dP.p, dQ.p, dM.p, &w);
+      if ( rc == HS_OK ) rc = hs_mirror_lower(0, dM.p, m1, m1);
+      if ( rc == HS_OK && hipMemcpy2DAsync(dL.p, (size_t) m * sizeof(double), dM.p + m1 + 1, (size_t) m1 * sizeof(double), (size_t) m * sizeof(double),
+               (size_t) m, hipMemcpyDeviceToDevice, 0) != hipSuccess ) rc = HS_ERR_HIP;
+      if ( rc == HS_OK && hipMemcpy2DAsync(dG.p, sizeof(double), dM.p + m1 + 1, (size_t) (m1 + 1) * sizeof(double), sizeof(double), (size_t) m,
+               hipMemcpyDeviceToDevice, 0) != hipSuccess ) rc = HS_ERR_HIP;
+   }
+   if ( hipDeviceSynchronize() != hipSuccess && rc == HS_OK ) rc = HS_ERR_HIP;
+   if ( used != NULL )
+   {
+      used[0] = hs_dgemm2_enable(1) - t2;
+      used[1] = hs_dgemm2_paired_taken() - t5;
+      used[2] = hs_gram_taken() - tg;
+   }
+   hs_schur_ws_free(&w);
+   HS_CALL( rc );
+   if ( staged && !*stages )
+      return HIPSDP_OK;
+   HS_CALL( dM.down(Mx, MM) ); HS_CALL( dL.down(Lm, (long long) m * m) );
+   return dG.down(dya, m);
+}
```

New measurement: 13.76 (median of 6 runs). No clear change (+0.7%).
